# howardlau1999/pytorch-ddp-template

Measured on NVIDIA H100. Metric: samples/sec (whole box, device-timed, max over ranks) for ResNet-50 DDP at 1/2/4/8 H100, higher is better.
Workload: dtype bf16; 1 GPU; model=resnet50, global_batch=32, per_gpu_batch=32, image_size=224, parallelism=dp1, loss=mse(dense one-hot target), optimizer=sgd lr1e-3 + clip_grad_norm 1000 + linear warmup/decay, transport=single, cuda_graph=True

## Files before the change

### b200ddp/csrc/conv_wgmma.cu

```cuda
#include "conv.h"

#include <cuda.h>
#include <mutex>
#include <unordered_map>
#include <vector>

#include "drv.h"
#include "tc_primitives.cuh"

namespace b200 {
namespace {
using namespace tc;

constexpr int BLOCK_K = 64;
constexpr int UMMA_K = 16;
constexpr int kThreads = 256;
constexpr int kMmaWarps = 4;
constexpr int kMaxRing = 12;
constexpr int kSlabBytes = 128 * 128;
constexpr int kStagingBytes = 2 * kSlabBytes;
constexpr int kBarrierBytes = 1024;
constexpr int kTrStride = 36;
constexpr int kStatsScratchBytes = 4 * 32 * kTrStride * 4;
__host__ __device__ constexpr int acc_stride(int block_n) { return block_n + 8; }
__host__ __device__ constexpr int acc_bytes(int block_n) { return 128 * acc_stride(block_n) * 4; }

struct TapGemmParams {
  int M_total, Kc, Nc;
  int R, S, pad;
  int mirror;
  int mode;
  int H, W;
  int BH, BI, tiles_h, Wp;
  int num_m_tiles, num_n_tiles;
  int dense_rows;
  int a_chunk_bytes;
  int KC, TB;
  int s_stage_bytes, s_stages, b_slot_bytes, b_stages;
  uint32_t a_tx_bytes;
  int set_base_offset;
  int b_tap_stride;
  int row_mul;
  int b_resident;
  int chunk_stride;
  float* col_stats;
  const __nv_bfloat16* addend;
  const __nv_bfloat16* bn_x;
  const uint8_t* bn_mask;
  const float* bn_mean;
  const float* bn_rstd;
  long long* dbg;
};

__device__ __forceinline__ void tma_load_4d(const CUtensorMap* map, uint64_t* bar, void* smem, int c0, int c1, int c2, int c3) {
  asm volatile(
      "cp.async.bulk.tensor.4d.shared::cluster.global.mbarrier::complete_tx::bytes [%0], [%1, {%3, %4, %5, %6}], [%2];"
      ::"r"(smem_u32(smem)), "l"(reinterpret_cast<uint64_t>(map)), "r"(smem_u32(bar)), "r"(c0), "r"(c1), "r"(c2), "r"(c3) : "memory");
}
__device__ __forceinline__ void bulk_wait_read_all() { asm volatile("cp.async.bulk.wait_group.read 0;" ::: "memory"); }
__device__ __forceinline__ void epi_bar_sync() { asm volatile("bar.sync 1, 128;" ::: "memory"); }

__device__ __forceinline__ uint64_t make_desc_rowoff(uint32_t addr, uint32_t lbo, uint32_t sbo, int set_base_offset) {
  uint64_t d = make_smem_desc(addr, lbo, sbo);
  if (set_base_offset) d |= (uint64_t)((addr >> 7) & 7u) << 49;
  return d;
}

__device__ __forceinline__ bool acc_row_to_dense(const TapGemmParams& p, int i, int* dense) {
  if (p.mode == 2) {
    const int h = i / p.Wp, w = i - h * p.Wp;
    *dense = h * p.W + w;
    return h < p.BH && w < p.W;
  }
  *dense = i;
  return i < p.dense_rows;
}

__device__ __forceinline__ float warp_column_sum32(const float* v, float* tr, int lane) {
#pragma unroll
  for (int q = 0; q < 8; ++q)
    *reinterpret_cast<float4*>(tr + lane * kTrStride + 4 * q) = make_float4(v[4 * q], v[4 * q + 1], v[4 * q + 2], v[4 * q + 3]);
  __syncwarp();
  float s = 0.f;
#pragma unroll
  for (int r = 0; r < 32; ++r) s += tr[r * kTrStride + lane];
  __syncwarp();
  return s;
}

__device__ __forceinline__ bool elect_one() {
  uint32_t pred;
  asm volatile("{\n\t.reg .pred P;\n\telect.sync _|P, 0xFFFFFFFF;\n\tselp.u32 %0, 1, 0, P;\n\t}" : "=r"(pred));
  return pred != 0;
}

template <int BLOCK_N, bool B_MN, int EPI>
__global__ void __launch_bounds__(kThreads, 1)
conv_tap_gemm_kernel(const __grid_constant__ CUtensorMap map_a, const __grid_constant__ CUtensorMap map_b,
                     const __grid_constant__ CUtensorMap map_d, const TapGemmParams p) {
  constexpr int kBBytes = BLOCK_N * BLOCK_K * 2;
  constexpr int kAccStride = acc_stride(BLOCK_N);
  extern __shared__ uint8_t smem_raw[];
  uint8_t* smem = reinterpret_cast<uint8_t*>((reinterpret_cast<uintptr_t>(smem_raw) + 1023) & ~uintptr_t(1023));
  uint8_t* s_ring = smem;
  uint8_t* b_ring = s_ring + p.s_stages * p.s_stage_bytes;
  uint8_t* staging = b_ring + p.b_stages * p.b_slot_bytes;
  [[maybe_unused]] float* stats_scratch = reinterpret_cast<float*>(staging + kStagingBytes);
  float* acc_smem = reinterpret_cast<float*>(staging + kStagingBytes + (EPI != 0 ? kStatsScratchBytes : 0));
  uint64_t* s_full = reinterpret_cast<uint64_t*>(reinterpret_cast<uint8_t*>(acc_smem) + acc_bytes(BLOCK_N));
  uint64_t* s_empty = s_full + kMaxRing;
  uint64_t* b_full = s_empty + kMaxRing;
  uint64_t* b_empty = b_full + kMaxRing;

  const int warp = threadIdx.x >> 5, lane = threadIdx.x & 31;
  const long long t_begin = clock64();
  const int num_tiles = p.num_m_tiles * p.num_n_tiles;
  const int cblocks = p.Kc / BLOCK_K;
  const int taps = p.R * p.S;
  const int chunks_per_tile = cblocks * taps;

  if (warp == 0 && lane == 0) { tma_prefetch_desc(&map_a); tma_prefetch_desc(&map_b); tma_prefetch_desc(&map_d); }
  if (warp == 1) {
    if (lane < kMaxRing) {
      mbar_init(&s_full[lane], (p.mode == 2 || p.b_resident) ? 1 : 2); mbar_init(&s_empty[lane], kMmaWarps);
      mbar_init(&b_full[lane], 1); mbar_init(&b_empty[lane], kMmaWarps);
    }
    asm volatile("fence.mbarrier_init.release.cluster;" ::: "memory");
  }
  __syncthreads();
#define B200_T0 if (dbg) t = clock64();
#define B200_T1(acc) if (dbg) acc += clock64() - t;

  if (warp == 0 || warp == 3) {
    const bool is_a = (warp == 0);
    int ss = 0, bs = 0;
    uint32_t sph = 0, bph = 0;
    long long d_w = 0, d_i = 0, t = 0;
    const bool dbg = p.dbg != nullptr && blockIdx.x == 0;
    if constexpr (!B_MN) {
      if (!is_a && p.b_resident) {
        if (elect_one()) {
          mbar_expect_tx(&b_full[0], (uint32_t)chunks_per_tile * kBBytes);
          int cb_i = 0, r_i = 0, s_i = 0;
          for (int q = 0; q < chunks_per_tile; ++q) {
            tma_load_2d(&map_b, &b_full[0], b_ring + q * kBBytes, (r_i * p.S + s_i) * p.b_tap_stride + cb_i * BLOCK_K, 0);
            if (++s_i == p.S) { s_i = 0; if (++r_i == p.R) { r_i = 0; ++cb_i; } }
          }
        }
        __syncwarp();
      }
    }
    for (int tile = blockIdx.x; tile < num_tiles; tile += gridDim.x) {
      const int mt = tile / p.num_n_tiles, nt = tile - mt * p.num_n_tiles;
      const int n0 = nt * BLOCK_N;
      int img0 = 0, h0 = 0;
      if (p.mode != 0) { img0 = (mt / p.tiles_h) * p.BI; h0 = (mt % p.tiles_h) * p.BH; }
      if (p.mode != 2) {
        if (!is_a && p.b_resident) continue;
        int cb = 0, r = 0, sx = 0;
        for (int q0 = 0; q0 < chunks_per_tile; q0 += p.KC) {
          B200_T0 mbar_wait(&s_empty[ss], sph ^ 1); B200_T1(d_w)
          B200_T0
          if (elect_one()) {
            uint8_t* dst = s_ring + ss * p.s_stage_bytes;
            int cb_i = cb, r_i = r, s_i = sx;
            if (is_a) {
              mbar_expect_tx(&s_full[ss], (uint32_t)p.KC * p.a_tx_bytes);
              for (int j = 0; j < p.KC; ++j) {
                if (p.mode == 0) {
                  tma_load_4d(&map_a, &s_full[ss], dst, cb_i * BLOCK_K, mt * 128, 0, 0);
                } else {
                  const int dh = p.mirror ? p.pad - r_i : r_i - p.pad, dw = p.mirror ? p.pad - s_i : s_i - p.pad;
                  tma_load_4d(&map_a, &s_full[ss], dst, cb_i * BLOCK_K, dw, h0 * p.row_mul + dh, img0);
                }
                dst += p.chunk_stride;
                if (++s_i == p.S) { s_i = 0; if (++r_i == p.R) { r_i = 0; ++cb_i; } }
              }
            } else {
              mbar_expect_tx(&s_full[ss], (uint32_t)p.KC * kBBytes);
              for (int j = 0; j < p.KC; ++j) {
                uint8_t* sb = dst + p.a_chunk_bytes;
                const int bcol = (r_i * p.S + s_i) * p.b_tap_stride;
                if constexpr (!B_MN) {
                  tma_load_2d(&map_b, &s_full[ss], sb, bcol + cb_i * BLOCK_K, n0);
                } else {
#pragma unroll
                  for (int c = 0; c < BLOCK_N / 64; ++c)
                    tma_load_2d(&map_b, &s_full[ss], sb + c * (64 * BLOCK_K * 2), bcol + n0 + 64 * c, cb_i * BLOCK_K);
                }
                dst += p.chunk_stride;
                if (++s_i == p.S) { s_i = 0; if (++r_i == p.R) { r_i = 0; ++cb_i; } }
              }
            }
          }
          __syncwarp();
          for (int j = 0; j < p.KC; ++j) { if (++sx == p.S) { sx = 0; if (++r == p.R) { r = 0; ++cb; } } }
          if (++ss == p.s_stages) { ss = 0; sph ^= 1; }
          B200_T1(d_i)
        }
      } else if (is_a) {
        for (int cb = 0; cb < cblocks; ++cb) {
          B200_T0 mbar_wait(&s_empty[ss], sph ^ 1); B200_T1(d_w)
          B200_T0
          if (elect_one()) {
            mbar_expect_tx(&s_full[ss], p.a_tx_bytes);
            tma_load_4d(&map_a, &s_full[ss], s_ring + ss * p.s_stage_bytes, cb * BLOCK_K, -p.pad, h0 - p.pad, img0);
          }
          __syncwarp();
          if (++ss == p.s_stages) { ss = 0; sph ^= 1; }
          B200_T1(d_i)
        }
      } else {
        for (int cb = 0; cb < cblocks; ++cb) {
          for (int tap0 = 0; tap0 < taps; tap0 += p.TB) {
            B200_T0 mbar_wait(&b_empty[bs], bph ^ 1); B200_T1(d_w)
            B200_T0
            if (elect_one()) {
              mbar_expect_tx(&b_full[bs], (uint32_t)p.TB * kBBytes);
              for (int j = 0; j < p.TB; ++j) {
                uint8_t* sb = b_ring + bs * p.b_slot_bytes + j * kBBytes;
                const int bcol = (tap0 + j) * p.b_tap_stride;
                if constexpr (!B_MN) {
                  tma_load_2d(&map_b, &b_full[bs], sb, bcol + cb * BLOCK_K, n0);
                } else {
#pragma unroll
                  for (int c = 0; c < BLOCK_N / 64; ++c)
                    tma_load_2d(&map_b, &b_full[bs], sb + c * (64 * BLOCK_K * 2), bcol + n0 + 64 * c, cb * BLOCK_K);
                }
              }
            }
            __syncwarp();
            if (++bs == p.b_stages) { bs = 0; bph ^= 1; }
            B200_T1(d_i)
          }
        }
      }
    }
    if (dbg && lane == 0) { p.dbg[is_a ? 0 : 2] = d_w; p.dbg[is_a ? 1 : 3] = d_i; }
  } else if (warp >= 4) {
    constexpr int kTB = B_MN ? 1 : 0;
    constexpr uint32_t kLboB = B_MN ? BLOCK_K * 128 : 16;
    constexpr uint32_t kStepB = B_MN ? UMMA_K * 128 : UMMA_K * 2;
    constexpr uint64_t kHalfA = (64 * 128) >> 4;
    const uint64_t a_desc0 = make_smem_desc(smem_u32(s_ring), 16, 1024);
    const uint64_t b_desc_s0 = make_smem_desc(smem_u32(s_ring), kLboB, 1024);
    const uint64_t b_desc_b0 = make_smem_desc(smem_u32(b_ring), kLboB, 1024);
    const int ew = warp - 4;
    const bool t0 = (ew == 0 && lane == 0);
    int ss = 0, bs = 0;
    uint32_t sph = 0, bph = 0, slab = 0;
    long long d_wf = 0, d_mma = 0, d_ep = 0, t = 0;
    const bool dbg = p.dbg != nullptr && blockIdx.x == 0 && t0;
    [[maybe_unused]] float st_s[BLOCK_N / 32], st_q[BLOCK_N / 32];
    constexpr bool STATS = (EPI != 0);
    [[maybe_unused]] float* tr = stats_scratch + ew * (32 * kTrStride);
    if constexpr (STATS) {
#pragma unroll
      for (int i = 0; i < BLOCK_N / 32; ++i) { st_s[i] = 0.f; st_q[i] = 0.f; }
    }
    if (p.b_resident) mbar_wait(&b_full[0], 0);
    for (int tile = blockIdx.x; tile < num_tiles; tile += gridDim.x) {
      WgAcc<BLOCK_N> acc;
      uint32_t acc_on = 0;
      if (p.mode != 2) {
        for (int q0 = 0; q0 < chunks_per_tile; q0 += p.KC) {
          B200_T0 mbar_wait(&s_full[ss], sph); B200_T1(d_wf)
          B200_T0
          wgmma_fence();
          uint32_t off = (uint32_t)(ss * p.s_stage_bytes);
          for (int j = 0; j < p.KC; ++j) {
            const uint64_t da = a_desc0 + (uint64_t)(off >> 4);
            const uint64_t db = p.b_resident ? b_desc_b0 + (uint64_t)(((uint32_t)(q0 + j) * (uint32_t)kBBytes) >> 4)
                                             : b_desc_s0 + (uint64_t)((off + p.a_chunk_bytes) >> 4);
#pragma unroll
            for (int k = 0; k < BLOCK_K / UMMA_K; ++k) {
              const uint64_t dak = da + (uint64_t)(k * ((UMMA_K * 2) >> 4));
              wgmma_tile<BLOCK_N, 0, kTB>(acc, dak, dak + kHalfA, db + (uint64_t)(k * (kStepB >> 4)), acc_on);
              acc_on = 1;
            }
            off += (uint32_t)p.chunk_stride;
          }
          wgmma_commit();
          wgmma_wait<0>();
          __syncwarp();
          if (lane == 0) mbar_arrive(&s_empty[ss]);
          if (++ss == p.s_stages) { ss = 0; sph ^= 1; }
          B200_T1(d_mma)
        }
      } else {
        for (int cb = 0; cb < cblocks; ++cb) {
          B200_T0 mbar_wait(&s_full[ss], sph); B200_T1(d_wf)
          const uint32_t a_off = (uint32_t)(ss * p.s_stage_bytes);
          for (int tap0 = 0; tap0 < taps; tap0 += p.TB) {
            B200_T0 mbar_wait(&b_full[bs], bph); B200_T1(d_wf)
            B200_T0
            wgmma_fence();
            int r = tap0 / p.S, sx = tap0 - r * p.S;
            for (int j = 0; j < p.TB; ++j) {
              const int rr = p.mirror ? (p.R - 1 - r) : r, sc = p.mirror ? (p.S - 1 - sx) : sx;
              const uint64_t da = make_desc_rowoff(smem_u32(s_ring) + a_off + (uint32_t)(rr * p.Wp + sc) * 128u, 16, 1024, p.set_base_offset);
              const uint64_t db = b_desc_b0 + (uint64_t)((uint32_t)(bs * p.b_slot_bytes + j * kBBytes) >> 4);
#pragma unroll
              for (int k = 0; k < BLOCK_K / UMMA_K; ++k) {
                const uint64_t dak = da + (uint64_t)(k * ((UMMA_K * 2) >> 4));
                wgmma_tile<BLOCK_N, 0, kTB>(acc, dak, dak + kHalfA, db + (uint64_t)(k * (kStepB >> 4)), acc_on);
                acc_on = 1;
              }
              if (++sx == p.S) { sx = 0; ++r; }
            }
            wgmma_commit();
            wgmma_wait<0>();
            __syncwarp();
            if (lane == 0) {
              mbar_arrive(&b_empty[bs]);
              if (tap0 + p.TB >= taps) mbar_arrive(&s_empty[ss]);
            }
            if (++bs == p.b_stages) { bs = 0; bph ^= 1; }
            B200_T1(d_mma)
          }
          if (++ss == p.s_stages) { ss = 0; sph ^= 1; }
        }
      }
      B200_T0
      const int mt = tile / p.num_n_tiles, nt = tile - mt * p.num_n_tiles;
      const int n0 = nt * BLOCK_N;
      int row0;
      if (p.mode == 0) row0 = mt * 128;
      else row0 = (((mt / p.tiles_h) * p.BI) * p.H + (mt % p.tiles_h) * p.BH) * p.W;
      int dense;
      bool valid = acc_row_to_dense(p, ew * 32 + lane, &dense);
      valid = valid && (row0 + dense < p.M_total);
      wg_bar_sync();
      acc_to_smem<BLOCK_N>(acc, acc_smem, kAccStride, threadIdx.x - 128);
      wg_bar_sync();
#pragma unroll
      for (int c = 0; c < BLOCK_N; c += 64) {
        if (n0 + c >= p.Nc) break;
        uint8_t* buf = staging + (slab & 1u) * kSlabBytes;
        const uint32_t buf_s = smem_u32(buf);
#pragma unroll
        for (int half = 0; half < 2; ++half) {
          uint32_t rr[32];
          acc_row_ld32(acc_smem, kAccStride, ew * 32 + lane, c + 32 * half, rr);
          if constexpr (EPI == 1) {
            float sv[32], qv[32];
#pragma unroll
            for (int i = 0; i < 32; ++i) {
              const float v = __bfloat162float(__float2bfloat16_rn(__uint_as_float(rr[i])));
              sv[i] = valid ? v : 0.f;
              qv[i] = sv[i] * sv[i];
            }
            const float cs = warp_column_sum32(sv, tr, lane);
            const float cq = warp_column_sum32(qv, tr, lane);
            const int ci = (c >> 5) + half;
#pragma unroll
            for (int i = 0; i < BLOCK_N / 32; ++i)
              if (i == ci) { st_s[i] += cs; st_q[i] += cq; }
          }
          if constexpr (EPI == 2) {
            const int col0 = n0 + c + 32 * half;
            const size_t grow = (size_t)(row0 + dense);
            float v[32];
#pragma unroll
            for (int i = 0; i < 32; ++i) v[i] = __uint_as_float(rr[i]);
            if (p.addend != nullptr && valid) {
              const uint4* ap = reinterpret_cast<const uint4*>(p.addend + grow * p.Nc + col0);
#pragma unroll
              for (int q = 0; q < 4; ++q) {
                const uint4 raw = __ldg(ap + q);
                const __nv_bfloat162* h = reinterpret_cast<const __nv_bfloat162*>(&raw);
#pragma unroll
                for (int j = 0; j < 4; ++j) { const float2 f = __bfloat1622float2(h[j]); v[8 * q + 2 * j] += f.x; v[8 * q + 2 * j + 1] += f.y; }
              }
            }
#pragma unroll
            for (int i = 0; i < 32; ++i) { v[i] = __bfloat162float(__float2bfloat16_rn(v[i])); rr[i] = __float_as_uint(v[i]); }
            if (p.bn_x != nullptr) {
              float sv[32], qv[32];
              uint32_t mk = 0xffffffffu;
              float xv[32];
              if (valid) {
                const uint4* xp = reinterpret_cast<const uint4*>(p.bn_x + grow * p.Nc + col0);
#pragma unroll
                for (int q = 0; q < 4; ++q) {
                  const uint4 raw = __ldg(xp + q);
                  const __nv_bfloat162* h = reinterpret_cast<const __nv_bfloat162*>(&raw);
#pragma unroll
                  for (int j = 0; j < 4; ++j) { const float2 f = __bfloat1622float2(h[j]); xv[8 * q + 2 * j] = f.x; xv[8 * q + 2 * j + 1] = f.y; }
                }
                if (p.bn_mask != nullptr) mk = __ldg(reinterpret_cast<const uint32_t*>(p.bn_mask + grow * (size_t)(p.Nc >> 3) + (col0 >> 3)));
              } else {
                mk = 0u;
#pragma unroll
                for (int i = 0; i < 32; ++i) xv[i] = 0.f;
              }
              const float my_mean = (col0 + lane < p.Nc) ? __ldg(p.bn_mean + col0 + lane) : 0.f;
              const float my_rstd = (col0 + lane < p.Nc) ? __ldg(p.bn_rstd + col0 + lane) : 0.f;
#pragma unroll
              for (int i = 0; i < 32; ++i) {
                const float mean_i = __shfl_sync(0xffffffffu, my_mean, i), rstd_i = __shfl_sync(0xffffffffu, my_rstd, i);
                const float dyp = ((mk >> i) & 1u) ? v[i] : 0.f;
                sv[i] = dyp;
                qv[i] = dyp * (xv[i] - mean_i) * rstd_i;
              }
              const float cs = warp_column_sum32(sv, tr, lane);
              const float cq = warp_column_sum32(qv, tr, lane);
              const int ci = (c >> 5) + half;
#pragma unroll
              for (int i = 0; i < BLOCK_N / 32; ++i)
                if (i == ci) { st_s[i] += cs; st_q[i] += cq; }
            }
          }
          if (valid) {
#pragma unroll
            for (int q = 0; q < 4; ++q) {
              __nv_bfloat162 h[4];
#pragma unroll
              for (int j = 0; j < 4; ++j) h[j] = __floats2bfloat162_rn(__uint_as_float(rr[8 * q + 2 * j]), __uint_as_float(rr[8 * q + 2 * j + 1]));
              const int chunk = half * 4 + q;
              const uint32_t* w = reinterpret_cast<const uint32_t*>(h);
              asm volatile("st.shared.v4.b32 [%0], {%1, %2, %3, %4};"
                           ::"r"(buf_s + (uint32_t)(dense * 128 + ((chunk ^ (dense & 7)) << 4))), "r"(w[0]), "r"(w[1]), "r"(w[2]), "r"(w[3]) : "memory");
            }
          }
        }
        fence_async_smem();
        if (t0) bulk_wait_read_all();
        epi_bar_sync();
        if (t0) { tma_store_2d(&map_d, buf, n0 + c, row0); bulk_commit(); }
        ++slab;
      }
      B200_T1(d_ep)
    }
    if (dbg) { p.dbg[5] = d_wf; p.dbg[6] = d_mma; p.dbg[9] = d_ep; }
    if (STATS && p.col_stats != nullptr) {
      float* comb = stats_scratch;
      epi_bar_sync();
#pragma unroll
      for (int i = 0; i < BLOCK_N / 32; ++i) {
        comb[(ew * 2 + 0) * BLOCK_N + 32 * i + lane] = st_s[i];
        comb[(ew * 2 + 1) * BLOCK_N + 32 * i + lane] = st_q[i];
      }
      epi_bar_sync();
      const int nt = blockIdx.x % p.num_n_tiles;
      const size_t g = (size_t)(blockIdx.x / p.num_n_tiles), G = (size_t)(gridDim.x / p.num_n_tiles);
      for (int j = ew * 32 + lane; j < 2 * BLOCK_N; j += 128) {
        const int which = j / BLOCK_N, cc = j - which * BLOCK_N;
        const int col = nt * BLOCK_N + cc;
        if (col < p.Nc) {
          const float v = ((comb[(0 * 2 + which) * BLOCK_N + cc] + comb[(1 * 2 + which) * BLOCK_N + cc]) + comb[(2 * 2 + which) * BLOCK_N + cc]) +
                          comb[(3 * 2 + which) * BLOCK_N + cc];
          p.col_stats[((size_t)which * G + g) * p.Nc + col] = v;
        }
      }
    }
    if (t0) bulk_wait_all();
  }

  __syncthreads();
  if (p.dbg != nullptr && blockIdx.x == 0 && threadIdx.x == 0) p.dbg[10] = clock64() - t_begin;
}
#undef B200_T0
#undef B200_T1

struct MapKey {
  const void* ptr; uint64_t d[4]; uint64_t s[3]; uint32_t b[4]; int rank;
  bool operator==(const MapKey& o) const {
    if (ptr != o.ptr || rank != o.rank) return false;
    for (int i = 0; i < 4; ++i) if (d[i] != o.d[i] || b[i] != o.b[i]) return false;
    for (int i = 0; i < 3; ++i) if (s[i] != o.s[i]) return false;
    return true;
  }
};
struct MapKeyHash {
  size_t operator()(const MapKey& k) const {
    size_t h = std::hash<const void*>()(k.ptr) ^ (size_t)k.rank;
    for (int i = 0; i < 4; ++i) h = (h * 1000003u) ^ (size_t)k.d[i] ^ ((size_t)k.b[i] << 20);
    for (int i = 0; i < 3; ++i) h = (h * 1000003u) ^ (size_t)k.s[i];
    return h;
  }
};

}

CUtensorMap conv_encode_map(const void* ptr, int rank, const uint64_t* dims, const uint64_t* strides, const uint32_t* box) {
  static std::mutex mu;
  static std::unordered_map<MapKey, CUtensorMap, MapKeyHash> cache;
  MapKey key{};
  key.ptr = ptr; key.rank = rank;
  for (int i = 0; i < rank; ++i) { key.d[i] = dims[i]; key.b[i] = box[i]; }
  for (int i = 0; i + 1 < rank; ++i) key.s[i] = strides[i];
  {
    std::lock_guard<std::mutex> g(mu);
    auto it = cache.find(key);
    if (it != cache.end()) return it->second;
  }
  auto& drv = Driver::get();
  if (!drv.TensorMapEncodeTiled) throw std::runtime_error("conv: cuTensorMapEncodeTiled unavailable");
  static thread_local bool ctx_bound = false;
  if (!ctx_bound) { B200_CUDA_CHECK(cudaFree(nullptr)); ctx_bound = true; }
  CUtensorMap map;
  cuuint64_t d[4], s[3];
  cuuint32_t b[4], es[4] = {1, 1, 1, 1};
  for (int i = 0; i < rank; ++i) { d[i] = dims[i]; b[i] = box[i]; }
  for (int i = 0; i + 1 < rank; ++i) s[i] = strides[i];
  B200_DRV_CHECK(drv.TensorMapEncodeTiled(&map, CU_TENSOR_MAP_DATA_TYPE_BFLOAT16, rank, const_cast<void*>(ptr), d, s, b, es,
                                          CU_TENSOR_MAP_INTERLEAVE_NONE, CU_TENSOR_MAP_SWIZZLE_128B, CU_TENSOR_MAP_L2_PROMOTION_L2_256B,
                                          CU_TENSOR_MAP_FLOAT_OOB_FILL_NONE));
  std::lock_guard<std::mutex> g(mu);
  if (cache.size() > 8192) cache.clear();
  cache.emplace(key, map);
  return map;
}

bool conv_tile_plan(int N, int H, int W, int R, int S, int want_mode, ConvTilePlan* plan) {
  ConvTilePlan pl;
  const int taps = R * S;
  if (taps == 1) {
    if (want_mode > 0) return false;
    pl.mode = 0;
    pl.num_m_tiles = ceil_div((long long)N * H * W, 128);
    pl.dense_rows = 128; pl.acc_rows = 128; pl.a_rows = 128;
    *plan = pl;
    return true;
  }
  if (R != 3 || S != 3) return false;
  auto halo = [&]() {
    const int Wp = W + 2;
    int bh = 0;
    for (int d = 1; d <= H; ++d)
      if (H % d == 0 && d * Wp <= 128 && (d + 2) * Wp <= 256 * 1) bh = d;
    if (bh == 0 || Wp > 256 || bh + 2 > 256) return false;
    pl.mode = 2; pl.BH = bh; pl.BI = 1; pl.tiles_h = H / bh; pl.Wp = Wp;
    pl.num_m_tiles = N * pl.tiles_h;
    pl.dense_rows = bh * W; pl.acc_rows = bh * Wp; pl.a_rows = (bh + 2) * Wp;
    return true;
  };
  auto patch = [&]() {
    if (W > 128) return false;
    int bh = 0;
    for (int d = 1; d <= H; ++d)
      if (H % d == 0 && W * d <= 128) bh = d;
    if (bh == 0) return false;
    int bi = 1;
    if (bh == H)
      for (int d = 1; d <= N; ++d)
        if (N % d == 0 && W * H * d <= 128) bi = d;
    pl.mode = 1; pl.BH = bh; pl.BI = bi; pl.tiles_h = H / bh; pl.Wp = W;
    pl.num_m_tiles = (N / bi) * pl.tiles_h;
    pl.dense_rows = W * bh * bi; pl.acc_rows = pl.dense_rows; pl.a_rows = pl.dense_rows;
    return true;
  };
  bool ok;
  if (want_mode == 1) ok = patch();
  else if (want_mode == 2) ok = halo();
  else ok = halo() || patch();
  if (!ok) return false;
  *plan = pl;
  return true;
}

int conv_grid_size(int num_m_tiles, int num_n_tiles, bool stats) {
  const long long tiles = (long long)num_m_tiles * num_n_tiles;
  int grid = tiles < kNumSMs ? (int)tiles : kNumSMs;
  if (stats && num_n_tiles > 1) {
    grid = (grid / num_n_tiles) * num_n_tiles;
    if (grid < num_n_tiles) grid = num_n_tiles;
  }
  return grid;
}

int conv_pick_block_n(int Nc, int num_m_tiles, int want) {
  (void)num_m_tiles;
  if (want == 256) return 128;
  if (want != 0) return want;
  return Nc % 128 != 0 ? 64 : 128;
}

int conv_stat_groups(int N, int H, int W, int Cin, int Cout, int R, int S, const ConvLaunchCfg& cfg) {
  ConvTilePlan pl;
  int mode = cfg.mode;
  if (mode < 0 && R == 3) mode = (Cin == 64) ? 2 : 1;
  if (!conv_tile_plan(N, H, W, R, S, mode, &pl)) return 0;
  const int bn = conv_pick_block_n(Cout, pl.num_m_tiles, cfg.block_n);
  const int nn = ceil_div(Cout, bn);
  return conv_grid_size(pl.num_m_tiles, nn, true) / nn;
}

namespace {

template <int BLOCK_N, bool B_MN, int EPI>
void launch_variant(const CUtensorMap& ma, const CUtensorMap& mb, const CUtensorMap& md, TapGemmParams p, int want_kc, cudaStream_t stream) {
  constexpr int kBBytes = BLOCK_N * BLOCK_K * 2;
  const int budget = 227 * 1024 - kStagingBytes - kBarrierBytes - 1024 - (EPI != 0 ? kStatsScratchBytes : 0) - acc_bytes(BLOCK_N);
  const int taps = p.R * p.S;
  if (p.mode != 2) {
    const int chunks_per_tile = (p.Kc / BLOCK_K) * taps;
    if (p.b_resident && (B_MN || p.num_n_tiles != 1)) throw std::runtime_error("conv: a resident filter needs a K-major filter and one n-tile");
    p.chunk_stride = p.a_chunk_bytes + (p.b_resident ? 0 : kBBytes);
    p.b_slot_bytes = p.b_resident ? chunks_per_tile * kBBytes : 0;
    p.b_stages = p.b_resident ? 1 : 0;
    const int chunk = p.chunk_stride;
    const int ring_budget = budget - p.b_stages * p.b_slot_bytes;
    int kc = want_kc > 0 ? want_kc : 2;
    while (kc > 1 && (chunks_per_tile % kc != 0 || ring_budget / (kc * chunk) < 3)) --kc;
    p.KC = kc; p.TB = 1;
    p.s_stage_bytes = kc * chunk;
    p.s_stages = ring_budget / p.s_stage_bytes;
    if (p.s_stages > kMaxRing) p.s_stages = kMaxRing;
    if (p.s_stages < 2) throw std::runtime_error("conv: shared memory budget exceeded");
  } else {
    p.KC = 1; p.chunk_stride = 0; p.b_resident = 0;
    p.s_stage_bytes = p.a_chunk_bytes;
    int s_st = 0, b_st = 0;
    for (int tb = 3; tb >= 1; tb -= 2) {
      if (tb == 3 && (3 * kBBytes > 48 * 1024 || taps % 3 != 0)) continue;
      p.TB = tb;
      p.b_slot_bytes = p.TB * kBBytes;
      const int groups = taps / p.TB;
      s_st = budget / (p.s_stage_bytes + groups * p.b_slot_bytes);
      if (s_st < 2) s_st = 2;
      if (s_st > kMaxRing) s_st = kMaxRing;
      b_st = (budget - s_st * p.s_stage_bytes) / p.b_slot_bytes;
      if (b_st > kMaxRing) b_st = kMaxRing;
      if (b_st >= 2) break;
    }
    if (b_st < 2) throw std::runtime_error("conv: shared memory budget exceeded");
    p.s_stages = s_st; p.b_stages = b_st;
  }
  const int smem = p.s_stages * p.s_stage_bytes + p.b_stages * p.b_slot_bytes + kStagingBytes + kBarrierBytes + 1024 + (EPI != 0 ? kStatsScratchBytes : 0) +
                   acc_bytes(BLOCK_N);
  auto kernel = conv_tap_gemm_kernel<BLOCK_N, B_MN, EPI>;
  static std::atomic<unsigned long long> configured{0};
  ensure_max_dynamic_smem(kernel, 227 * 1024, configured);
  const int grid = conv_grid_size(p.num_m_tiles, p.num_n_tiles, EPI != 0);
  kernel<<<grid, kThreads, smem, stream>>>(ma, mb, md, p);
  B200_CUDA_CHECK(cudaGetLastError()); B200_COUNT_LAUNCH(1);
}

}

void launch_conv_tap_gemm(const void* a, const void* w, void* d, int N, int H, int W, int Cin, int Cout, int R, int S, bool dgrad,
                          const ConvLaunchCfg& cfg, float* col_stats, cudaStream_t stream, const ConvBwdFusion* fuse) {
  const int Kc = dgrad ? Cout : Cin, Nc = dgrad ? Cin : Cout;
  if (Kc % BLOCK_K != 0 || Nc % 64 != 0) throw std::runtime_error("conv: channel counts must be multiples of 64");
  if (R != S || (R != 1 && R != 3)) throw std::runtime_error("conv: 1x1 or 3x3 filters");
  if (dgrad && fuse == nullptr && col_stats != nullptr) throw std::runtime_error("conv: column statistics ride on the forward pass only");
  if (fuse != nullptr && !dgrad) throw std::runtime_error("conv: the BatchNorm-backward fusion rides on the data gradient");
  if (fuse != nullptr && fuse->bn_x != nullptr && col_stats == nullptr) throw std::runtime_error("conv: fused BatchNorm backward needs the partial-sum workspace");
  ConvTilePlan pl;
  int mode = cfg.mode;
  if (mode < 0 && R == 3) mode = (Kc == 64) ? 2 : 1;
  if (!conv_tile_plan(N, H, W, R, S, mode, &pl)) throw std::runtime_error("conv: no tile plan for this geometry");
  const long long M_total = (long long)N * H * W;
  TapGemmParams p{};
  p.M_total = (int)M_total; p.Kc = Kc; p.Nc = Nc;
  p.R = R; p.S = S; p.pad = (R - 1) / 2;
  p.mirror = dgrad ? 1 : 0;
  p.mode = pl.mode;
  p.H = H; p.W = W; p.BH = pl.BH; p.BI = pl.BI; p.tiles_h = pl.tiles_h; p.Wp = pl.Wp;
  p.num_m_tiles = pl.num_m_tiles;
  p.dense_rows = pl.dense_rows;
  p.a_tx_bytes = (uint32_t)(pl.a_rows * 128);
  p.a_chunk_bytes = ((pl.a_rows * 128 + 1023) / 1024) * 1024;
  if (p.a_chunk_bytes < 128 * 128) p.a_chunk_bytes = 128 * 128;
  p.set_base_offset = cfg.set_base_offset;
  p.b_tap_stride = Cin;
  p.row_mul = 1;
  p.b_resident = 0;
  p.col_stats = col_stats;
  p.addend = fuse ? reinterpret_cast<const __nv_bfloat16*>(fuse->addend) : nullptr;
  p.bn_x = fuse ? reinterpret_cast<const __nv_bfloat16*>(fuse->bn_x) : nullptr;
  p.bn_mask = fuse ? reinterpret_cast<const uint8_t*>(fuse->bn_mask) : nullptr;
  p.bn_mean = fuse ? fuse->bn_mean : nullptr;
  p.bn_rstd = fuse ? fuse->bn_rstd : nullptr;
  p.dbg = reinterpret_cast<long long*>(cfg.debug_counters);
  const int block_n = conv_pick_block_n(Nc, pl.num_m_tiles, cfg.block_n);
  if (block_n != 64 && block_n != 128) throw std::runtime_error("conv: block_n must be 0 (auto), 64, 128 or 256 (runs as two 128-wide n-tiles)");
  p.num_n_tiles = ceil_div(Nc, block_n);

  CUtensorMap ma;
  if (pl.mode == 0) {
    uint64_t dm[4] = {(uint64_t)Kc, (uint64_t)M_total, 1, 1};
    uint64_t st[3] = {(uint64_t)Kc * 2, (uint64_t)Kc * 2 * (uint64_t)M_total, (uint64_t)Kc * 2 * (uint64_t)M_total};
    uint32_t bx[4] = {64, 128, 1, 1};
    ma = conv_encode_map(a, 4, dm, st, bx);
  } else {
    uint64_t dm[4] = {(uint64_t)Kc, (uint64_t)W, (uint64_t)H, (uint64_t)N};
    uint64_t st[3] = {(uint64_t)Kc * 2, (uint64_t)W * Kc * 2, (uint64_t)H * W * Kc * 2};
    uint32_t bx[4] = {64, (uint32_t)(pl.mode == 2 ? pl.Wp : W), (uint32_t)(pl.mode == 2 ? pl.BH + 2 : pl.BH), (uint32_t)pl.BI};
    ma = conv_encode_map(a, 4, dm, st, bx);
  }
  CUtensorMap mb;
  {
    uint64_t dm[2] = {(uint64_t)R * S * Cin, (uint64_t)Cout};
    uint64_t st[1] = {(uint64_t)R * S * Cin * 2};
    uint32_t bx[2] = {64, (uint32_t)(dgrad ? 64 : block_n)};
    mb = conv_encode_map(w, 2, dm, st, bx);
  }
  CUtensorMap md;
  {
    uint64_t dm[2] = {(uint64_t)Nc, (uint64_t)M_total};
    uint64_t st[1] = {(uint64_t)Nc * 2};
    uint32_t bx[2] = {64, (uint32_t)pl.dense_rows};
    md = conv_encode_map(d, 2, dm, st, bx);
  }
#define B200_CONV_DISPATCH(BN)                                                                         \
  if (block_n == BN) {                                                                                 \
    if (dgrad && fuse != nullptr) launch_variant<BN, true, 2>(ma, mb, md, p, cfg.kc, stream);          \
    else if (dgrad) launch_variant<BN, true, 0>(ma, mb, md, p, cfg.kc, stream);                        \
    else if (col_stats != nullptr) launch_variant<BN, false, 1>(ma, mb, md, p, cfg.kc, stream);        \
    else launch_variant<BN, false, 0>(ma, mb, md, p, cfg.kc, stream);                                  \
    return;                                                                                            \
  }
  B200_CONV_DISPATCH(64)
  B200_CONV_DISPATCH(128)
#undef B200_CONV_DISPATCH
}

int stem_stat_groups(int N, int H, int W) {
  StemGeom g;
  if (!stem_geom(H, W, &g)) return 0;
  return conv_grid_size(N * g.Ho, 1, true);
}

void launch_stem_conv_fprop(const void* xp, const void* w2, void* y, int N, int H, int W, int Cout, float* col_stats, bool resident_filter,
                            void* debug_counters, cudaStream_t stream) {
  StemGeom g;
  if (!stem_geom(H, W, &g)) throw std::runtime_error("stem conv: unsupported image size");
  if (Cout != 64) throw std::runtime_error("stem conv: 64 output channels");
  const long long M_total = (long long)N * g.Ho * g.Wo;
  TapGemmParams p{};
  p.M_total = (int)M_total; p.Kc = 64; p.Nc = Cout;
  p.R = kStemTaps; p.S = 1; p.pad = 0; p.mirror = 0;
  p.mode = 1;
  p.H = g.Ho; p.W = g.Wo; p.BH = 1; p.BI = 1; p.tiles_h = g.Ho; p.Wp = g.Wo;
  p.num_m_tiles = N * g.Ho;
  p.num_n_tiles = 1;
  p.dense_rows = g.Wo;
  p.a_tx_bytes = (uint32_t)(g.Wo * 128);
  p.a_chunk_bytes = 128 * 128;
  p.b_tap_stride = 64;
  p.row_mul = 1;
  p.b_resident = resident_filter ? 1 : 0;
  p.col_stats = col_stats;
  p.dbg = reinterpret_cast<long long*>(debug_counters);
  const uint64_t row_pitch = (uint64_t)g.Wp * 16;
  CUtensorMap ma, mb, md;
  {
    uint64_t dm[4] = {64, (uint64_t)g.Wo, (uint64_t)g.Hp2, (uint64_t)N};
    uint64_t st[3] = {32, row_pitch, row_pitch * (uint64_t)g.Hp2};
    uint32_t bx[4] = {64, (uint32_t)g.Wo, 1, 1};
    ma = conv_encode_map(xp, 4, dm, st, bx);
  }
  {
    uint64_t dm[2] = {(uint64_t)kStemK, (uint64_t)Cout};
    uint64_t st[1] = {(uint64_t)kStemK * 2};
    uint32_t bx[2] = {64, 64};
    mb = conv_encode_map(w2, 2, dm, st, bx);
  }
  {
    uint64_t dm[2] = {(uint64_t)Cout, (uint64_t)M_total};
    uint64_t st[1] = {(uint64_t)Cout * 2};
    uint32_t bx[2] = {64, (uint32_t)g.Wo};
    md = conv_encode_map(y, 2, dm, st, bx);
  }
  if (col_stats != nullptr) launch_variant<64, false, 1>(ma, mb, md, p, 0, stream);
  else launch_variant<64, false, 0>(ma, mb, md, p, 0, stream);
}

}
```

### b200ddp/csrc/conv_wgrad_wgmma.cu

```cuda
#include "conv.h"

#include <cuda.h>

#include "drv.h"
#include "tc_primitives.cuh"

namespace b200 {

CUtensorMap conv_encode_map(const void* ptr, int rank, const uint64_t* dims, const uint64_t* strides, const uint32_t* box);

namespace {
using namespace tc;

constexpr int UMMA_K = 16;
constexpr int kThreads = 256;
constexpr int kMmaWarps = 4;
constexpr int kMaxRing = 12;
constexpr int kBarrierBytes = 1024;

struct WgradParams {
  int Cout, Cin, R, S, pad;
  int mode;
  int H, W, BH, BI, tiles_h;
  int row_mul;
  int KB;
  int num_kblocks;
  int MB, TG, tile_n;
  int m_groups, n_tiles, tap_groups, split;
  int a_slot_bytes, b_slot_bytes, a_stages, b_stages;
  float* partial;
};

__device__ __forceinline__ void tma_load_4d(const CUtensorMap* map, uint64_t* bar, void* smem, int c0, int c1, int c2, int c3) {
  asm volatile(
      "cp.async.bulk.tensor.4d.shared::cluster.global.mbarrier::complete_tx::bytes [%0], [%1, {%3, %4, %5, %6}], [%2];"
      ::"r"(smem_u32(smem)), "l"(reinterpret_cast<uint64_t>(map)), "r"(smem_u32(bar)), "r"(c0), "r"(c1), "r"(c2), "r"(c3) : "memory");
}

__device__ __forceinline__ bool elect_one() {
  uint32_t pred;
  asm volatile("{\n\t.reg .pred P;\n\telect.sync _|P, 0xFFFFFFFF;\n\tselp.u32 %0, 1, 0, P;\n\t}" : "=r"(pred));
  return pred != 0;
}

template <int N>
__device__ __forceinline__ void store_half_rows(const float (&h)[N / 2], float* out, size_t ld, int rows_valid, int cols_valid, bool zero, int wg_thread) {
  const int r0 = (wg_thread >> 5) * 16 + ((wg_thread & 31) >> 2), c0 = 2 * (wg_thread & 3);
#pragma unroll
  for (int j = 0; j < N / 8; ++j) {
#pragma unroll
    for (int hi = 0; hi < 2; ++hi) {
      const int r = r0 + 8 * hi, c = 8 * j + c0;
      if (r < rows_valid && c < cols_valid)
        *reinterpret_cast<float2*>(out + (size_t)r * ld + c) = zero ? make_float2(0.f, 0.f) : make_float2(h[4 * j + 2 * hi], h[4 * j + 2 * hi + 1]);
    }
  }
}

template <int TILE_N>
__global__ void __launch_bounds__(kThreads, 1)
conv_wgrad_kernel(const __grid_constant__ CUtensorMap map_dy, const __grid_constant__ CUtensorMap map_x, const WgradParams p) {
  extern __shared__ uint8_t smem_raw[];
  uint8_t* smem = reinterpret_cast<uint8_t*>((reinterpret_cast<uintptr_t>(smem_raw) + 1023) & ~uintptr_t(1023));
  uint8_t* a_ring = smem;
  uint8_t* b_ring = a_ring + p.a_stages * p.a_slot_bytes;
  uint64_t* a_full = reinterpret_cast<uint64_t*>(b_ring + p.b_stages * p.b_slot_bytes);
  uint64_t* a_empty = a_full + kMaxRing;
  uint64_t* b_full = a_empty + kMaxRing;
  uint64_t* b_empty = b_full + kMaxRing;

  const int warp = threadIdx.x >> 5, lane = threadIdx.x & 31;
  const int unit = blockIdx.x;
  const int grp = unit / p.split, sp = unit - grp * p.split;
  const int tg = grp % p.tap_groups;
  const int nt = (grp / p.tap_groups) % p.n_tiles;
  const int mg = grp / (p.tap_groups * p.n_tiles);
  const int taps = p.R * p.S;
  const int tap0 = tg * p.TG;
  const int ntaps = min(p.TG, taps - tap0);
  const int co0 = mg * p.MB * 128;
  const int ci0 = nt * p.tile_n;
  const int kb0 = (int)(((long long)p.num_kblocks * sp) / p.split);
  const int kb1 = (int)(((long long)p.num_kblocks * (sp + 1)) / p.split);
  const int chunk_bytes = p.KB * 128;
  const int a_chunks = p.MB * 2, b_chunks = p.tile_n / 64;

  if (warp == 0 && lane == 0) { tma_prefetch_desc(&map_dy); tma_prefetch_desc(&map_x); }
  if (warp == 1) {
    if (lane < kMaxRing) { mbar_init(&a_full[lane], 1); mbar_init(&a_empty[lane], kMmaWarps); mbar_init(&b_full[lane], 1); mbar_init(&b_empty[lane], kMmaWarps); }
    asm volatile("fence.mbarrier_init.release.cluster;" ::: "memory");
  }
  __syncthreads();

  if (warp == 0) {
    int as = 0;
    uint32_t aph = 0;
    for (int kb = kb0; kb < kb1; ++kb) {
      int c1 = 0, c2 = 0, c3 = 0;
      if (p.mode == 0) c1 = kb * p.KB;
      else { c3 = (kb / p.tiles_h) * p.BI; c2 = (kb % p.tiles_h) * p.BH; }
      mbar_wait(&a_empty[as], aph ^ 1);
      if (elect_one()) {
        mbar_expect_tx(&a_full[as], (uint32_t)(a_chunks * chunk_bytes));
        for (int j = 0; j < a_chunks; ++j)
          tma_load_4d(&map_dy, &a_full[as], a_ring + as * p.a_slot_bytes + j * chunk_bytes, co0 + 64 * j, c1, c2, c3);
      }
      __syncwarp();
      if (++as == p.a_stages) { as = 0; aph ^= 1; }
    }
  } else if (warp == 3) {
    int bs = 0;
    uint32_t bph = 0;
    for (int kb = kb0; kb < kb1; ++kb) {
      int c1 = 0, c2 = 0, c3 = 0;
      if (p.mode == 0) c1 = kb * p.KB;
      else { c3 = (kb / p.tiles_h) * p.BI; c2 = (kb % p.tiles_h) * p.BH; }
      int r = tap0 / p.S, sx = tap0 - r * p.S;
      for (int t = 0; t < ntaps; ++t) {
        mbar_wait(&b_empty[bs], bph ^ 1);
        if (elect_one()) {
          mbar_expect_tx(&b_full[bs], (uint32_t)(b_chunks * chunk_bytes));
          for (int j = 0; j < b_chunks; ++j)
            tma_load_4d(&map_x, &b_full[bs], b_ring + bs * p.b_slot_bytes + j * chunk_bytes, ci0 + 64 * j,
                        p.mode == 0 ? c1 : sx - p.pad, p.mode == 0 ? 0 : c2 * p.row_mul + r - p.pad, c3);
        }
        __syncwarp();
        if (++sx == p.S) { sx = 0; ++r; }
        if (++bs == p.b_stages) { bs = 0; bph ^= 1; }
      }
    }
  } else if (warp >= 4) {
    const uint32_t lbo = (uint32_t)chunk_bytes;
    const int ksteps = p.KB / UMMA_K;
    const uint64_t a_desc0 = make_smem_desc(smem_u32(a_ring), lbo, 1024);
    const uint64_t b_desc0 = make_smem_desc(smem_u32(b_ring), lbo, 1024);
    const uint64_t half_a = (uint64_t)(chunk_bytes >> 4);
    WgAcc<TILE_N> acc;
    int as = 0, bs = 0;
    uint32_t aph = 0, bph = 0;
    for (int kb = kb0; kb < kb1; ++kb) {
      mbar_wait(&a_full[as], aph);
      for (int t = 0; t < ntaps; ++t) {
        mbar_wait(&b_full[bs], bph);
        wgmma_fence();
        const uint64_t da0 = a_desc0 + (uint64_t)((uint32_t)(as * p.a_slot_bytes) >> 4);
        const uint64_t db0 = b_desc0 + (uint64_t)((uint32_t)(bs * p.b_slot_bytes) >> 4);
        for (int k = 0; k < ksteps; ++k) {
          const uint64_t step = (uint64_t)(k * ((UMMA_K * 128) >> 4));
          wgmma_tile<TILE_N, 1, 1>(acc, da0 + step, da0 + half_a + step, db0 + step, (kb != kb0 || k != 0) ? 1u : 0u);
        }
        wgmma_commit();
        wgmma_wait<0>();
        __syncwarp();
        if (lane == 0) {
          mbar_arrive(&b_empty[bs]);
          if (t == ntaps - 1) mbar_arrive(&a_empty[as]);
        }
        if (++bs == p.b_stages) { bs = 0; bph ^= 1; }
      }
      if (++as == p.a_stages) { as = 0; aph ^= 1; }
    }
    const int row_len = taps * p.Cin;
    float* out = p.partial + (size_t)sp * p.Cout * row_len + (size_t)co0 * row_len + (size_t)tap0 * p.Cin + ci0;
#pragma unroll
    for (int half = 0; half < 2; ++half)
      store_half_rows<TILE_N>(acc.h[half], out + (size_t)(64 * half) * row_len, (size_t)row_len, p.Cout - co0 - 64 * half, p.Cin - ci0,
                              kb1 <= kb0, threadIdx.x - 128);
  }
}

__global__ void __launch_bounds__(256) conv_wgrad_reduce_kernel(const float* __restrict__ partial, __nv_bfloat16* __restrict__ out, size_t n, int split) {
  __shared__ float sm[8][32][9];
  const int v = threadIdx.x & 31, sl = threadIdx.x >> 5;
  const size_t e = ((size_t)blockIdx.x * 32 + v) * 8;
  float acc[8] = {0.f, 0.f, 0.f, 0.f, 0.f, 0.f, 0.f, 0.f};
  if (e < n) {
#pragma unroll 2
    for (int s = sl; s < split; s += 8) {
      const float4 lo = __ldcg(reinterpret_cast<const float4*>(partial + (size_t)s * n + e));
      const float4 hi = __ldcg(reinterpret_cast<const float4*>(partial + (size_t)s * n + e + 4));
      acc[0] += lo.x; acc[1] += lo.y; acc[2] += lo.z; acc[3] += lo.w;
      acc[4] += hi.x; acc[5] += hi.y; acc[6] += hi.z; acc[7] += hi.w;
    }
  }
#pragma unroll
  for (int i = 0; i < 8; ++i) sm[sl][v][i] = acc[i];
  __syncthreads();
  if (sl == 0 && e < n) {
#pragma unroll
    for (int j = 1; j < 8; ++j)
#pragma unroll
      for (int i = 0; i < 8; ++i) acc[i] += sm[j][v][i];
    *reinterpret_cast<Bf16x8*>(out + e) = pack8(acc);
  }
}

struct WgradPlan {
  WgradParams p;
  int smem;
  int grid;
};

bool wgrad_plan(int N, int H, int W, int Cin, int Cout, int R, int S, const WgradCfg& cfg, WgradPlan* out) {
  if (Cin % 64 != 0 || Cout % 64 != 0 || R != S || (R != 1 && R != 3)) return false;
  WgradParams p{};
  p.Cout = Cout; p.Cin = Cin; p.R = R; p.S = S; p.pad = (R - 1) / 2;
  p.H = H; p.W = W; p.row_mul = 1;
  const int taps = R * S;
  if (taps == 1) {
    p.mode = 0; p.KB = 64;
    p.num_kblocks = ceil_div((long long)N * H * W, p.KB);
    p.BH = p.BI = p.tiles_h = 0;
  } else {
    p.mode = 1;
    int bh = 0, bi = 1;
    for (int d = 1; d <= 16 && bh == 0; ++d) {
      for (int i = 1; i <= (d >= H ? 4 : 1); ++i) {
        const int kb = W * d * i;
        if (kb % 16 == 0 && kb >= 96 && kb <= 128) { bh = d; bi = i; break; }
      }
    }
    if (bh == 0) {
      for (int d = 1; d <= H + 15 && bh == 0; ++d)
        if ((W * d) % 16 == 0 && W * d <= 128) bh = d;
      if (bh == 0) return false;
    }
    if (bi > 1 && N % bi != 0) return false;
    p.BH = bh; p.BI = bi; p.tiles_h = ceil_div(H, bh);
    p.KB = W * bh * bi;
    p.num_kblocks = (N / bi) * p.tiles_h;
  }
  const int MB = 1, TG = 1;
  int tile_n = Cin < 128 ? Cin : 128;
  if (cfg.tile_m > 0 && cfg.tile_m != 128) return false;
  if (cfg.tile_n > 0) tile_n = cfg.tile_n;
  if ((tile_n != 64 && tile_n != 128) || tile_n > Cin) return false;
  p.MB = MB; p.TG = TG; p.tile_n = tile_n;
  p.m_groups = ceil_div(Cout, 128 * MB);
  p.n_tiles = ceil_div(Cin, tile_n);
  p.tap_groups = ceil_div(taps, TG);
  const int groups = p.m_groups * p.n_tiles * p.tap_groups;
  int split = cfg.split > 0 ? cfg.split : kNumSMs / groups;
  if (split < 1) split = 1;
  if (split > p.num_kblocks) split = p.num_kblocks;
  p.split = split;
  const int chunk = p.KB * 128;
  p.a_slot_bytes = MB * 2 * chunk;
  p.b_slot_bytes = (tile_n / 64) * chunk;
  const int budget = 227 * 1024 - kBarrierBytes - 1024;
  int ast = budget / (p.a_slot_bytes + TG * p.b_slot_bytes);
  if (ast < 1) ast = 1;
  if (ast > kMaxRing) ast = kMaxRing;
  int bst = (budget - ast * p.a_slot_bytes) / p.b_slot_bytes;
  if (bst > kMaxRing) bst = kMaxRing;
  if (bst < 1) return false;
  p.a_stages = ast;
  p.b_stages = bst;
  out->p = p;
  out->smem = p.a_stages * p.a_slot_bytes + p.b_stages * p.b_slot_bytes + kBarrierBytes + 1024;
  out->grid = groups * split;
  return true;
}

void launch_wgrad_kernel(const CUtensorMap& mdy, const CUtensorMap& mx, const WgradPlan& pl, cudaStream_t stream) {
  if (pl.p.tile_n == 64) {
    static std::atomic<unsigned long long> configured{0};
    ensure_max_dynamic_smem(conv_wgrad_kernel<64>, 227 * 1024, configured);
    conv_wgrad_kernel<64><<<pl.grid, kThreads, pl.smem, stream>>>(mdy, mx, pl.p);
  } else {
    static std::atomic<unsigned long long> configured{0};
    ensure_max_dynamic_smem(conv_wgrad_kernel<128>, 227 * 1024, configured);
    conv_wgrad_kernel<128><<<pl.grid, kThreads, pl.smem, stream>>>(mdy, mx, pl.p);
  }
}

}

size_t conv_wgrad_workspace_floats(int N, int H, int W, int Cin, int Cout, int R, int S, const WgradCfg& cfg) {
  WgradPlan pl;
  if (!wgrad_plan(N, H, W, Cin, Cout, R, S, cfg, &pl)) return 0;
  return (size_t)pl.p.split * Cout * R * S * Cin;
}

void launch_conv_wgrad(const void* dy, const void* x, void* dw, int N, int H, int W, int Cin, int Cout, int R, int S,
                       const WgradCfg& cfg, float* workspace, cudaStream_t stream) {
  WgradPlan pl;
  if (!wgrad_plan(N, H, W, Cin, Cout, R, S, cfg, &pl)) throw std::runtime_error("conv wgrad: unsupported geometry / tiling");
  WgradParams& p = pl.p;
  p.partial = workspace;
  const long long M_total = (long long)N * H * W;
  CUtensorMap mdy, mx;
  if (p.mode == 0) {
    uint64_t dd[4] = {(uint64_t)Cout, (uint64_t)M_total, 1, 1};
    uint64_t ds[3] = {(uint64_t)Cout * 2, (uint64_t)Cout * 2 * (uint64_t)M_total, (uint64_t)Cout * 2 * (uint64_t)M_total};
    uint32_t bx[4] = {64, (uint32_t)p.KB, 1, 1};
    mdy = conv_encode_map(dy, 4, dd, ds, bx);
    uint64_t xd[4] = {(uint64_t)Cin, (uint64_t)M_total, 1, 1};
    uint64_t xs[3] = {(uint64_t)Cin * 2, (uint64_t)Cin * 2 * (uint64_t)M_total, (uint64_t)Cin * 2 * (uint64_t)M_total};
    mx = conv_encode_map(x, 4, xd, xs, bx);
  } else {
    uint32_t bx[4] = {64, (uint32_t)W, (uint32_t)p.BH, (uint32_t)p.BI};
    uint64_t dd[4] = {(uint64_t)Cout, (uint64_t)W, (uint64_t)H, (uint64_t)N};
    uint64_t ds[3] = {(uint64_t)Cout * 2, (uint64_t)W * Cout * 2, (uint64_t)H * W * Cout * 2};
    mdy = conv_encode_map(dy, 4, dd, ds, bx);
    uint64_t xd[4] = {(uint64_t)Cin, (uint64_t)W, (uint64_t)H, (uint64_t)N};
    uint64_t xs[3] = {(uint64_t)Cin * 2, (uint64_t)W * Cin * 2, (uint64_t)H * W * Cin * 2};
    mx = conv_encode_map(x, 4, xd, xs, bx);
  }
  launch_wgrad_kernel(mdy, mx, pl, stream);
  B200_CUDA_CHECK(cudaGetLastError());
  const size_t n = (size_t)Cout * R * S * Cin;
  conv_wgrad_reduce_kernel<<<(unsigned)((n / 8 + 31) / 32), 256, 0, stream>>>(workspace, reinterpret_cast<__nv_bfloat16*>(dw), n, p.split);
  B200_CUDA_CHECK(cudaGetLastError()); B200_COUNT_LAUNCH(2);
}

namespace {

struct StemWgradParams {
  int KB;
  int Ho, num_kblocks, split, Cout;
  int chunk_bytes, a_stages, b_stages;
  float* partial;
};
constexpr int kStemGroups = kStemTaps / 2;

__global__ void __launch_bounds__(kThreads, 1)
stem_wgrad_kernel(const __grid_constant__ CUtensorMap map_x, const __grid_constant__ CUtensorMap map_dy, const StemWgradParams p) {
  extern __shared__ uint8_t smem_raw[];
  uint8_t* smem = reinterpret_cast<uint8_t*>((reinterpret_cast<uintptr_t>(smem_raw) + 1023) & ~uintptr_t(1023));
  const int a_slot_bytes = 2 * p.chunk_bytes;
  uint8_t* a_ring = smem;
  uint8_t* b_ring = a_ring + p.a_stages * a_slot_bytes;
  uint64_t* a_full = reinterpret_cast<uint64_t*>(b_ring + p.b_stages * p.chunk_bytes);
  uint64_t* a_empty = a_full + kMaxRing;
  uint64_t* b_full = a_empty + kMaxRing;
  uint64_t* b_empty = b_full + kMaxRing;

  const int warp = threadIdx.x >> 5, lane = threadIdx.x & 31;
  const int sp = blockIdx.x;
  const int kb0 = (int)(((long long)p.num_kblocks * sp) / p.split);
  const int kb1 = (int)(((long long)p.num_kblocks * (sp + 1)) / p.split);

  if (warp == 0 && lane == 0) { tma_prefetch_desc(&map_x); tma_prefetch_desc(&map_dy); }
  if (warp == 1) {
    if (lane < kMaxRing) { mbar_init(&a_full[lane], 1); mbar_init(&a_empty[lane], kMmaWarps); mbar_init(&b_full[lane], 1); mbar_init(&b_empty[lane], kMmaWarps); }
    asm volatile("fence.mbarrier_init.release.cluster;" ::: "memory");
  }
  __syncthreads();

  if (warp == 0) {
    int as = 0;
    uint32_t aph = 0;
    for (int kb = kb0; kb < kb1; ++kb) {
      const int img = kb / p.Ho, oh = kb - img * p.Ho;
      for (int g = 0; g < kStemGroups; ++g) {
        mbar_wait(&a_empty[as], aph ^ 1);
        if (elect_one()) {
          uint8_t* dst = a_ring + as * a_slot_bytes;
          mbar_expect_tx(&a_full[as], (uint32_t)(2 * p.chunk_bytes));
          tma_load_4d(&map_x, &a_full[as], dst, 0, 0, oh + 2 * g, img);
          tma_load_4d(&map_x, &a_full[as], dst + p.chunk_bytes, 0, 0, oh + 2 * g + 1, img);
        }
        __syncwarp();
        if (++as == p.a_stages) { as = 0; aph ^= 1; }
      }
    }
  } else if (warp == 3) {
    int bs = 0;
    uint32_t bph = 0;
    for (int kb = kb0; kb < kb1; ++kb) {
      const int img = kb / p.Ho, oh = kb - img * p.Ho;
      mbar_wait(&b_empty[bs], bph ^ 1);
      if (elect_one()) {
        mbar_expect_tx(&b_full[bs], (uint32_t)p.chunk_bytes);
        tma_load_4d(&map_dy, &b_full[bs], b_ring + bs * p.chunk_bytes, 0, 0, oh, img);
      }
      __syncwarp();
      if (++bs == p.b_stages) { bs = 0; bph ^= 1; }
    }
  } else if (warp >= 4) {
    const int ksteps = p.KB / UMMA_K;
    const uint64_t a_desc0 = make_smem_desc(smem_u32(a_ring), (uint32_t)p.chunk_bytes, 1024);
    const uint64_t b_desc0 = make_smem_desc(smem_u32(b_ring), (uint32_t)p.chunk_bytes, 1024);
    const uint64_t half_a = (uint64_t)(p.chunk_bytes >> 4);
    WgAcc<64> acc[kStemGroups];
    int as = 0, bs = 0;
    uint32_t aph = 0, bph = 0;
    for (int kb = kb0; kb < kb1; ++kb) {
      mbar_wait(&b_full[bs], bph);
#pragma unroll
      for (int g = 0; g < kStemGroups; ++g) {
        mbar_wait(&a_full[as], aph);
        wgmma_fence();
        const uint64_t da0 = a_desc0 + (uint64_t)((uint32_t)(as * a_slot_bytes) >> 4);
        const uint64_t db0 = b_desc0 + (uint64_t)((uint32_t)(bs * p.chunk_bytes) >> 4);
        for (int k = 0; k < ksteps; ++k) {
          const uint64_t step = (uint64_t)(k * ((UMMA_K * 128) >> 4));
          wgmma_tile<64, 1, 1>(acc[g], da0 + step, da0 + half_a + step, db0 + step, (kb != kb0 || k != 0) ? 1u : 0u);
        }
        wgmma_commit();
        wgmma_wait<0>();
        __syncwarp();
        if (lane == 0) {
          mbar_arrive(&a_empty[as]);
          if (g == kStemGroups - 1) mbar_arrive(&b_empty[bs]);
        }
        if (++as == p.a_stages) { as = 0; aph ^= 1; }
      }
      if (++bs == p.b_stages) { bs = 0; bph ^= 1; }
    }
    float* base = p.partial + (size_t)sp * kStemK * p.Cout;
#pragma unroll
    for (int g = 0; g < kStemGroups; ++g)
#pragma unroll
      for (int half = 0; half < 2; ++half)
        store_half_rows<64>(acc[g].h[half], base + (size_t)(g * 128 + 64 * half) * p.Cout, (size_t)p.Cout, 64, p.Cout, kb1 <= kb0, threadIdx.x - 128);
  }
}

bool stem_generic_plan(int N, int H, int W, int Cout, WgradPlan* out) {
  StemGeom g;
  if (!stem_geom(H, W, &g) || Cout != 64) return false;
  WgradParams p{};
  p.Cout = Cout; p.Cin = 64; p.R = kStemTaps; p.S = 1; p.pad = 0;
  p.mode = 1; p.H = g.Ho; p.W = g.Wo; p.BH = 1; p.BI = 1; p.tiles_h = g.Ho; p.row_mul = 1;
  p.KB = g.Wo;
  p.num_kblocks = N * g.Ho;
  p.MB = 1; p.TG = 1; p.tile_n = 64;
  p.m_groups = 1; p.n_tiles = 1; p.tap_groups = kStemTaps;
  p.split = kNumSMs / kStemTaps;
  if (p.split > p.num_kblocks) p.split = p.num_kblocks;
  const int chunk = p.KB * 128;
  p.a_slot_bytes = 2 * chunk;
  p.b_slot_bytes = chunk;
  const int budget = 227 * 1024 - kBarrierBytes - 1024;
  p.a_stages = 3;
  int bst = (budget - p.a_stages * p.a_slot_bytes) / p.b_slot_bytes;
  if (bst > kMaxRing) bst = kMaxRing;
  if (bst < 2) return false;
  p.b_stages = bst;
  out->p = p;
  out->smem = p.a_stages * p.a_slot_bytes + p.b_stages * p.b_slot_bytes + kBarrierBytes + 1024;
  out->grid = p.tap_groups * p.split;
  return true;
}

bool stem_dedicated_plan(int N, int H, int W, int Cout, StemWgradParams* out, int* smem) {
  StemGeom g;
  if (!stem_geom(H, W, &g) || Cout != 64) return false;
  StemWgradParams p{};
  p.KB = g.Wo; p.Ho = g.Ho; p.Cout = Cout;
  p.num_kblocks = N * g.Ho;
  p.split = p.num_kblocks < kNumSMs ? p.num_kblocks : kNumSMs;
  p.chunk_bytes = p.KB * 128;
  const int budget = 227 * 1024 - kBarrierBytes - 1024;
  p.b_stages = 3;
  int ast = (budget - p.b_stages * p.chunk_bytes) / (2 * p.chunk_bytes);
  if (ast > kMaxRing) ast = kMaxRing;
  if (ast < 2) return false;
  p.a_stages = ast;
  *out = p;
  *smem = p.a_stages * 2 * p.chunk_bytes + p.b_stages * p.chunk_bytes + kBarrierBytes + 1024;
  return true;
}
}

size_t stem_wgrad_workspace_floats(int N, int H, int W, int Cout, int variant) {
  if (variant == 1) {
    WgradPlan pl;
    if (!stem_generic_plan(N, H, W, Cout, &pl)) return 0;
    return (size_t)pl.p.split * Cout * kStemK;
  }
  StemWgradParams p; int smem;
  if (!stem_dedicated_plan(N, H, W, Cout, &p, &smem)) return 0;
  return (size_t)p.split * Cout * kStemK;
}

void launch_stem_conv_wgrad(const void* dy, const void* xp, void* dw2, int N, int H, int W, int Cout, int variant, float* workspace,
                            cudaStream_t stream) {
  StemGeom g;
  if (!stem_geom(H, W, &g)) throw std::runtime_error("stem wgrad: unsupported geometry");
  CUtensorMap mdy, mx;
  uint32_t bx[4] = {64, (uint32_t)g.Wo, 1, 1};
  {
    uint64_t dd[4] = {(uint64_t)Cout, (uint64_t)g.Wo, (uint64_t)g.Ho, (uint64_t)N};
    uint64_t ds[3] = {(uint64_t)Cout * 2, (uint64_t)g.Wo * Cout * 2, (uint64_t)g.Ho * g.Wo * Cout * 2};
    mdy = conv_encode_map(dy, 4, dd, ds, bx);
  }
  {
    const uint64_t row_pitch = (uint64_t)g.Wp * 16;
    uint64_t xd[4] = {64, (uint64_t)g.Wo, (uint64_t)g.Hp2, (uint64_t)N};
    uint64_t xs[3] = {32, row_pitch, row_pitch * (uint64_t)g.Hp2};
    mx = conv_encode_map(xp, 4, xd, xs, bx);
  }
  const size_t n = (size_t)Cout * kStemK;
  int split = 0;
  if (variant == 1) {
    WgradPlan pl;
    if (!stem_generic_plan(N, H, W, Cout, &pl)) throw std::runtime_error("stem wgrad: unsupported geometry");
    pl.p.partial = workspace;
    launch_wgrad_kernel(mdy, mx, pl, stream);
    split = pl.p.split;
  } else {
    StemWgradParams p; int smem;
    if (!stem_dedicated_plan(N, H, W, Cout, &p, &smem)) throw std::runtime_error("stem wgrad: unsupported geometry");
    p.partial = workspace;
    static std::atomic<unsigned long long> configured{0};
    ensure_max_dynamic_smem(stem_wgrad_kernel, 227 * 1024, configured);
    stem_wgrad_kernel<<<p.split, kThreads, smem, stream>>>(mx, mdy, p);
    split = p.split;
  }
  B200_CUDA_CHECK(cudaGetLastError());
  conv_wgrad_reduce_kernel<<<(unsigned)((n / 8 + 31) / 32), 256, 0, stream>>>(workspace, reinterpret_cast<__nv_bfloat16*>(dw2), n, split);
  B200_CUDA_CHECK(cudaGetLastError()); B200_COUNT_LAUNCH(2);
}

}
```

### b200ddp/models/resnet.py

```python
from __future__ import annotations

import os
from typing import List

import torch
import torch.nn as nn

from ..ops import Conv3x3, FusedBatchNormAct2d, Linear, MaxPool3x3s2, PointwiseConv2d, StemConv7x7
from ..ops.bottleneck import bottleneck_forward, bottleneck_native_ok


class Bottleneck(nn.Module):
    expansion = 4

    def __init__(self, inplanes: int, planes: int, stride: int = 1, downsample: nn.Module | None = None):
        super().__init__()
        self.conv1 = PointwiseConv2d(inplanes, planes)
        self.bn1 = FusedBatchNormAct2d(planes, relu=True)
        self.conv2 = Conv3x3(planes, planes, stride=stride)
        self.bn2 = FusedBatchNormAct2d(planes, relu=True)
        self.conv3 = PointwiseConv2d(planes, planes * self.expansion)
        self.bn3 = FusedBatchNormAct2d(planes * self.expansion, relu=True)
        self.downsample = downsample

    def forward(self, x):
        if os.environ.get("B200DDP_BLOCK_FUSE", "0") == "1" and bottleneck_native_ok(self, x):
            return bottleneck_forward(self, x)
        if self.downsample is None:
            identity = x
        else:
            y, part = self.downsample[0].forward_with_stats(x)
            identity = self.downsample[1](y, partials=part)
        y, part = self.conv1.forward_with_stats(x)
        out = self.bn1(y, partials=part)
        y, part = self.conv2.forward_with_stats(out)
        out = self.bn2(y, partials=part)
        y, part = self.conv3.forward_with_stats(out)
        return self.bn3(y, residual=identity, partials=part)


class ResNet(nn.Module):
    def __init__(self, layers: List[int], num_classes: int = 1000, zero_init_residual: bool = False):
        super().__init__()
        self.inplanes = 64
        self.conv1 = StemConv7x7(3, 64)
        self.bn1 = FusedBatchNormAct2d(64, relu=True)
        self.maxpool = MaxPool3x3s2()
        self.layer1 = self._make_layer(64, layers[0], 1)
        self.layer2 = self._make_layer(128, layers[1], 2)
        self.layer3 = self._make_layer(256, layers[2], 2)
        self.layer4 = self._make_layer(512, layers[3], 2)
        self.avgpool = nn.AdaptiveAvgPool2d((1, 1))
        self.fc = Linear(512 * Bottleneck.expansion, num_classes)
        for m in self.modules():
            if isinstance(m, nn.Conv2d):
                nn.init.kaiming_normal_(m.weight, mode="fan_out", nonlinearity="relu")
            elif isinstance(m, nn.BatchNorm2d):
                nn.init.ones_(m.weight)
                nn.init.zeros_(m.bias)
        if zero_init_residual:
            for m in self.modules():
                if isinstance(m, Bottleneck):
                    nn.init.zeros_(m.bn3.weight)

    def _make_layer(self, planes: int, blocks: int, stride: int) -> nn.Sequential:
        downsample = None
        if stride != 1 or self.inplanes != planes * Bottleneck.expansion:
            downsample = nn.Sequential(PointwiseConv2d(self.inplanes, planes * Bottleneck.expansion, stride=stride),
                                       FusedBatchNormAct2d(planes * Bottleneck.expansion))
        mods = [Bottleneck(self.inplanes, planes, stride, downsample)]
        self.inplanes = planes * Bottleneck.expansion
        mods += [Bottleneck(self.inplanes, planes) for _ in range(1, blocks)]
        return nn.Sequential(*mods)

    def forward(self, x):
        if self.training:
            y, part = self.conv1.forward_with_stats(x)
        else:
            y, part = self.conv1(x), None
        x = self.maxpool(self.bn1(y, partials=part))
        x = self.layer4(self.layer3(self.layer2(self.layer1(x))))
        x = torch.flatten(self.avgpool(x), 1)
        return self.fc(x)


def resnet50(num_classes: int = 1000, **kw) -> ResNet:
    return ResNet([3, 4, 6, 3], num_classes, **kw)


def resnet152(num_classes: int = 1000, **kw) -> ResNet:
    return ResNet([3, 8, 36, 3], num_classes, **kw)
```

### b200ddp/ops/functional.py

```python
from __future__ import annotations

import math
import os
from typing import Optional

import torch
import torch.nn.functional as F

from .. import _ext

EPI_NONE, EPI_BIAS, EPI_BIAS_RELU, EPI_BIAS_GELU = 0, 1, 2, 3
_ACT_TO_EPI = {None: EPI_BIAS, "relu": EPI_BIAS_RELU, "gelu": EPI_BIAS_GELU}
_GELU_TANH = {"gelu": False, "gelu_tanh": True}


def _gelu_tanh_grad(p: torch.Tensor) -> torch.Tensor:
    k = math.sqrt(2.0 / math.pi)
    t = torch.tanh(k * (p + 0.044715 * p * p * p))
    return 0.5 * (1.0 + t) + 0.5 * p * (1.0 - t * t) * k * (1.0 + 3.0 * 0.044715 * p * p)


def _C():
    return _ext.get()


def _tc_ok(M: int, N: int, K: int) -> bool:
    return K % 8 == 0 and N % 8 == 0 and M % 8 == 0


class _LinearTC(torch.autograd.Function):

    @staticmethod
    def forward(ctx, x, weight, bias, activation):
        C = _C()
        x2 = x.reshape(-1, x.shape[-1])
        if not x2.is_contiguous():
            x2 = x2.contiguous()
        if bias is None and activation is not None:
            raise ValueError("fused activation needs a bias (use bias=True)")
        if activation in _GELU_TANH:
            pre = C.gemm_nt(x2, weight, bias, EPI_BIAS, None)
            y = C.gelu_fwd(pre, _GELU_TANH[activation])
            ctx.save_for_backward(x2, weight, pre)
        else:
            y = C.gemm_nt(x2, weight, bias, _ACT_TO_EPI[activation] if bias is not None else EPI_NONE, None)
            ctx.save_for_backward(x2, weight, y if activation == "relu" else None)
        ctx.activation = activation
        ctx.has_bias = bias is not None
        ctx.x_shape = x.shape
        return y.view(*x.shape[:-1], weight.shape[0])

    @staticmethod
    def backward(ctx, dy):
        C = _C()
        x2, weight, aux = ctx.saved_tensors
        dy2 = dy.reshape(-1, dy.shape[-1])
        if ctx.activation == "relu":
            dy2 = dy2 * (aux > 0).to(dy2.dtype)
        elif ctx.activation in _GELU_TANH:
            dy2 = C.gelu_bwd(dy2.contiguous(), aux, _GELU_TANH[ctx.activation])
        if not dy2.is_contiguous():
            dy2 = dy2.contiguous()
        dx = dw = db = None
        if ctx.needs_input_grad[0]:
            dx = C.gemm(dy2, weight, None, False, True, EPI_NONE, False, None).view(ctx.x_shape)
        if ctx.needs_input_grad[1]:
            dw = C.gemm(dy2, x2, None, True, True, EPI_NONE, False, None)
        if ctx.has_bias and ctx.needs_input_grad[2]:
            db = dy2.sum(0)
        return dx, dw, db, None


class _LinearSmall(torch.autograd.Function):

    @staticmethod
    def forward(ctx, x, weight, bias, relu):
        C = _C()
        xc = x.contiguous()
        y = C.small_linear_fwd(xc, weight.contiguous(), bias, bool(relu))
        ctx.save_for_backward(xc, weight, y)
        ctx.relu = bool(relu)
        ctx.has_bias = bias is not None
        return y

    @staticmethod
    def backward(ctx, dy):
        C = _C()
        x, weight, y = ctx.saved_tensors
        dx, dw, db = C.small_linear_bwd(dy, x, weight.contiguous(), y, ctx.relu, ctx.needs_input_grad[0], ctx.has_bias)
        return (dx if ctx.needs_input_grad[0] else None), dw, (db if ctx.has_bias else None), None


FP8_FORMATS = {"e4m3": (torch.float8_e4m3fn, 448.0), "e5m2": (torch.float8_e5m2, 57344.0)}


def fp8_scale(amax: float, fmt: str) -> float:
    fmax = FP8_FORMATS[fmt][1]
    if not (amax > 0.0) or not math.isfinite(amax):
        return 1.0
    ma, ea = math.frexp(amax)
    mf, ef = math.frexp(fmax)
    e = ef - ea - (1 if ma > mf else 0)
    return math.ldexp(1.0, min(max(e, -126), 127))


def fp8_quantize_reference(t: torch.Tensor, fmt: str):
    s = fp8_scale(float(t.detach().abs().max().float()) if t.numel() else 0.0, fmt)
    return (t.detach().float() * s).to(FP8_FORMATS[fmt][0]), s


def _fp8_round_trip(t: torch.Tensor, fmt: str) -> torch.Tensor:
    q, s = fp8_quantize_reference(t, fmt)
    return q.float() / s


def _fp8_check(x2: torch.Tensor, weight: torch.Tensor, bias: Optional[torch.Tensor], need_transpose_x: bool) -> None:
    M, K = x2.shape
    N = weight.shape[0]
    if x2.dtype != torch.bfloat16 or weight.dtype != torch.bfloat16 or (bias is not None and bias.dtype != torch.bfloat16):
        raise ValueError(f"fp8 linear on CUDA needs bf16 input, weight and bias, got {x2.dtype} x {weight.dtype} "
                         f"(input {tuple(x2.shape)}, weight {tuple(weight.shape)})")
    if K % 16 or N % 16:
        raise ValueError(f"fp8 linear needs in_features and out_features divisible by 16, got weight {tuple(weight.shape)}")
    if need_transpose_x and M % 16:
        raise ValueError(f"fp8 linear backward needs the row count divisible by 16 (the weight gradient reduces over rows "
                         f"of a transposed FP8 copy), got input {tuple(x2.shape)}")


class _LinearFP8(torch.autograd.Function):

    @staticmethod
    def forward(ctx, x, weight, bias, activation, grad_enabled):
        x2 = x.reshape(-1, x.shape[-1])
        if not x2.is_contiguous():
            x2 = x2.contiguous()
        if bias is None and activation is not None:
            raise ValueError("fused activation needs a bias (use bias=True)")
        need_dx, need_dw = grad_enabled and ctx.needs_input_grad[0], grad_enabled and ctx.needs_input_grad[1]
        ctx.activation = activation
        ctx.has_bias = bias is not None
        ctx.x_shape = x.shape
        if x.is_cuda:
            C = _C()
            _fp8_check(x2, weight, bias, need_dw)
            xq, xqt, xs, _ = C.fp8_quantize(x2, "e4m3", need_dw, False)
            wq, wqt, ws, _ = C.fp8_quantize(weight.contiguous(), "e4m3", need_dx, False)
            if activation in _GELU_TANH:
                pre = C.gemm_fp8(xq, wq, xs, ws, bias, EPI_BIAS)
                y = C.gelu_fwd(pre, _GELU_TANH[activation])
            else:
                pre = None
                y = C.gemm_fp8(xq, wq, xs, ws, bias, _ACT_TO_EPI[activation] if bias is not None else EPI_NONE)
                if activation == "relu":
                    pre = y
            ctx.save_for_backward(xqt, xs, wqt, ws, pre)
        else:
            xd = _fp8_round_trip(x2, "e4m3")
            wd = _fp8_round_trip(weight, "e4m3")
            acc = xd @ wd.t()
            if bias is not None:
                acc = acc + bias.float()
            pre = acc.to(x.dtype)
            if activation == "gelu":
                y = F.gelu(pre.float()).to(x.dtype)
            elif activation == "gelu_tanh":
                y = F.gelu(pre.float(), approximate="tanh").to(x.dtype)
            elif activation == "relu":
                y = F.relu(pre)
            else:
                y = pre
            ctx.save_for_backward(xd, wd, pre if activation is not None else None)
            ctx.dtypes = (x.dtype, weight.dtype, bias.dtype if bias is not None else None)
        return y.view(*x.shape[:-1], weight.shape[0])

    @staticmethod
    def backward(ctx, dy):
        dy2 = dy.reshape(-1, dy.shape[-1])
        dx = dw = db = None
        if dy.is_cuda:
            C = _C()
            xqt, xs, wqt, ws, aux = ctx.saved_tensors
            if ctx.activation == "relu":
                dy2 = dy2 * (aux > 0).to(dy2.dtype)
            elif ctx.activation in _GELU_TANH:
                dy2 = C.gelu_bwd(dy2.contiguous(), aux, _GELU_TANH[ctx.activation])
            if not dy2.is_contiguous():
                dy2 = dy2.contiguous()
            if dy2.shape[0] % 16:
                raise ValueError(f"fp8 linear backward needs the row count divisible by 16, got gradient {tuple(dy2.shape)}")
            need_db = ctx.has_bias and ctx.needs_input_grad[2]
            dyq, dyqt, dys, colsum = C.fp8_quantize(dy2, "e5m2", ctx.needs_input_grad[1], need_db)
            if ctx.needs_input_grad[0]:
                dx = C.gemm_fp8(dyq, wqt, dys, ws, None, EPI_NONE).view(ctx.x_shape)
            if ctx.needs_input_grad[1]:
                dw = C.gemm_fp8(dyqt, xqt, dys, xs, None, EPI_NONE)
            if need_db:
                db = colsum.to(dy.dtype)
        else:
            xd, wd, aux = ctx.saved_tensors
            x_dtype, w_dtype, b_dtype = ctx.dtypes
            if ctx.activation == "relu":
                dy2 = dy2 * (aux > 0).to(dy2.dtype)
            elif ctx.activation == "gelu":
                p = aux.float()
                dgelu = 0.5 * (1.0 + torch.erf(p * math.sqrt(0.5))) + p * torch.exp(-0.5 * p * p) / math.sqrt(2.0 * math.pi)
                dy2 = (dy2.float() * dgelu).to(dy.dtype)
            elif ctx.activation == "gelu_tanh":
                dy2 = (dy2.float() * _gelu_tanh_grad(aux.float())).to(dy.dtype)
            dyd = _fp8_round_trip(dy2, "e5m2")
            if ctx.needs_input_grad[0]:
                dx = (dyd @ wd).to(x_dtype).view(ctx.x_shape)
            if ctx.needs_input_grad[1]:
                dw = (dyd.t() @ xd).to(w_dtype)
            if ctx.has_bias and ctx.needs_input_grad[2]:
                db = dy2.float().sum(0).to(b_dtype)
        return dx, dw, db, None, None


def linear(x: torch.Tensor, weight: torch.Tensor, bias: Optional[torch.Tensor] = None,
           activation: Optional[str] = None, fp8: bool = False) -> torch.Tensor:
    if fp8:
        return _LinearFP8.apply(x, weight, bias, activation, torch.is_grad_enabled())
    if x.is_cuda:
        N, K = weight.shape
        M = x.numel() // K
        if x.dtype == torch.bfloat16 and weight.dtype == torch.bfloat16 and _tc_ok(M, N, K) \
                and (bias is not None or activation is None) and os.environ.get("B200DDP_DISABLE_TC", "0") != "1":
            return _LinearTC.apply(x, weight, bias, activation)
        if x.dtype == torch.float32 and weight.dtype == torch.float32 and N * (K + 1) * 4 <= 48 * 1024 and M * N * 4 <= 48 * 1024 \
                and activation in (None, "relu"):
            return _LinearSmall.apply(x, weight, bias, activation == "relu")
        _C()
        y = F.linear(x, weight, bias)
    else:
        y = F.linear(x, weight, bias)
    if activation == "relu":
        y = F.relu(y)
    elif activation == "gelu":
        y = F.gelu(y)
    elif activation == "gelu_tanh":
        y = F.gelu(y, approximate="tanh")
    return y


ATTENTION_HEAD_DIM = 64
ATTENTION_SEQ_MULTIPLE = 128


def _key_mask(seq_lens: torch.Tensor, S: int, device) -> torch.Tensor:
    lens = seq_lens.to(device=device, dtype=torch.long).clamp(0, S)
    return torch.arange(S, device=device)[None, :] < lens[:, None]


def attention_reference(qkv: torch.Tensor, seq_lens: torch.Tensor, heads: int) -> torch.Tensor:
    return _masked_attention_reference(qkv, _key_mask(seq_lens, qkv.shape[1], qkv.device)[:, None, None, :], heads)


def _masked_attention_reference(qkv: torch.Tensor, keep: torch.Tensor, heads: int) -> torch.Tensor:
    B, S, W = qkv.shape
    hidden = W // 3
    hd = hidden // heads
    ct = torch.promote_types(qkv.dtype, torch.float32)
    q, k, v = (t.to(ct).reshape(B, S, heads, hd).transpose(1, 2) for t in qkv.split(hidden, dim=-1))
    scores = (q @ k.transpose(-1, -2)) * (1.0 / math.sqrt(hd))
    p = torch.softmax(scores.masked_fill(~keep, torch.finfo(ct).min), dim=-1) * keep
    return (p @ v).transpose(1, 2).reshape(B, S, hidden).to(qkv.dtype)


def _attention_check(qkv: torch.Tensor, seq_lens: torch.Tensor, heads: int) -> None:
    _qkv_check(qkv, heads)
    B = qkv.shape[0]
    if seq_lens.dim() != 1 or seq_lens.shape[0] != B or seq_lens.is_floating_point() or seq_lens.is_complex():
        raise ValueError(f"attention needs integer seq_lens [B] = [{B}], got {seq_lens.dtype} {tuple(seq_lens.shape)}")


def _qkv_check(qkv: torch.Tensor, heads: int) -> None:
    if qkv.dim() != 3 or qkv.shape[-1] % 3:
        raise ValueError(f"attention needs qkv [B, S, 3 * hidden], got {tuple(qkv.shape)}")
    B, S, W = qkv.shape
    if heads < 1 or (W // 3) % heads or (W // 3) // heads != ATTENTION_HEAD_DIM:
        raise ValueError(f"attention on CUDA supports head dim {ATTENTION_HEAD_DIM} only, got hidden {W // 3} over {heads} heads")
    if qkv.dtype != torch.bfloat16:
        raise ValueError(f"attention on CUDA needs bf16 qkv, got {qkv.dtype}")
    if S % ATTENTION_SEQ_MULTIPLE or S == 0:
        raise ValueError(f"attention on CUDA needs the sequence length to be a multiple of {ATTENTION_SEQ_MULTIPLE}, got {S}")
    if not qkv.is_contiguous():
        raise ValueError("attention on CUDA needs a contiguous qkv (the fused projection's output)")


_ATTENTION_MODES = {
    "key_padding": ("attention_fwd", "attention_bwd", lambda: attention_reference),
    "packed": ("packed_attention_fwd", "packed_attention_bwd", lambda: packed_attention_reference),
    "causal": ("causal_attention_fwd", "causal_attention_bwd", lambda: causal_attention_reference),
}


class _Attention(torch.autograd.Function):

    @staticmethod
    def forward(ctx, qkv, mask, heads, mode):
        ctx.heads, ctx.mode = heads, mode
        if qkv.is_cuda:
            B, S, W = qkv.shape
            m = mask.to(device=qkv.device, dtype=torch.int32).contiguous()
            o, lse = getattr(_C(), _ATTENTION_MODES[mode][0])(qkv.view(B * S, W), m, heads)
            ctx.save_for_backward(qkv, o, lse, m)
            return o.view(B, S, W // 3)
        ctx.save_for_backward(qkv, mask)
        return _ATTENTION_MODES[mode][2]()(qkv, mask, heads)

    @staticmethod
    def backward(ctx, dy):
        if dy.is_cuda:
            qkv, o, lse, m = ctx.saved_tensors
            B, S, W = qkv.shape
            do = dy.reshape(B * S, W // 3).to(torch.bfloat16).contiguous()
            if do.data_ptr() % 16:
                do = do.clone()
            dqkv = getattr(_C(), _ATTENTION_MODES[ctx.mode][1])(do, qkv.view(B * S, W), o, lse, m, ctx.heads)
            return dqkv.view(B, S, W), None, None, None
        qkv, mask = ctx.saved_tensors
        ref = _ATTENTION_MODES[ctx.mode][2]()
        with torch.enable_grad():
            x = qkv.detach().requires_grad_(True)
            (g,) = torch.autograd.grad(ref(x, mask, ctx.heads), x, dy)
        return g, None, None, None


def attention(qkv: torch.Tensor, seq_lens: torch.Tensor, heads: int) -> torch.Tensor:
    if qkv.is_cuda:
        _attention_check(qkv, seq_lens, heads)
    return _Attention.apply(qkv, seq_lens, heads, "key_padding")


def document_bounds(input_ids: torch.Tensor, cls_token_id: Optional[int], pad_token_id: Optional[int]):
    B, S = input_ids.shape
    pos = torch.arange(S, device=input_ids.device).expand(B, S)
    if pad_token_id is None:
        lens = torch.full((B, 1), S, device=input_ids.device, dtype=torch.long)
    else:
        lens = (input_ids != pad_token_id).sum(1, keepdim=True)
    valid = pos < lens
    is_start = (pos == 0) if cls_token_id is None else (input_ids == cls_token_id) | (pos == 0)
    is_start = is_start & valid
    start = torch.where(is_start, pos, 0).cummax(1).values
    nxt = torch.where(is_start, pos, S)[:, 1:]
    nxt = torch.cat([nxt, torch.full((B, 1), S, device=pos.device, dtype=pos.dtype)], 1).flip(1).cummin(1).values.flip(1)
    end = torch.minimum(nxt, lens)
    bounds = torch.stack([torch.where(valid, start, 0), torch.where(valid, end, 0)], -1).to(torch.int32)
    return bounds, torch.where(valid, pos - start, 0)


def _bounds_mask(bounds: torch.Tensor, S: int, device) -> torch.Tensor:
    b = bounds.to(device=device, dtype=torch.long).reshape(-1, S, 2)
    start = b[..., 0].clamp(0, S)
    end = torch.maximum(b[..., 1].clamp(max=S), start)
    j = torch.arange(S, device=device)
    return (j >= start[..., None]) & (j < end[..., None])


def packed_attention_reference(qkv: torch.Tensor, bounds: torch.Tensor, heads: int) -> torch.Tensor:
    return _masked_attention_reference(qkv, _bounds_mask(bounds, qkv.shape[1], qkv.device)[:, None], heads)


def packed_attention(qkv: torch.Tensor, bounds: torch.Tensor, heads: int) -> torch.Tensor:
    if qkv.is_cuda:
        _qkv_check(qkv, heads)
        _bounds_check(qkv, bounds, "packed attention")
    return _Attention.apply(qkv, bounds, heads, "packed")


def _bounds_check(qkv: torch.Tensor, bounds: torch.Tensor, who: str) -> None:
    B, S = qkv.shape[:2]
    if tuple(bounds.shape) != (B, S, 2) or bounds.is_floating_point() or bounds.is_complex():
        raise ValueError(f"{who} needs integer bounds [B, S, 2] = [{B}, {S}, 2], got {bounds.dtype} {tuple(bounds.shape)}")


def _causal_mask(bounds: torch.Tensor, S: int, device) -> torch.Tensor:
    i = torch.arange(S, device=device)
    return _bounds_mask(bounds, S, device) & (i[None, :] <= i[:, None])


def causal_attention_reference(qkv: torch.Tensor, bounds: torch.Tensor, heads: int, kv_heads: Optional[int] = None) -> torch.Tensor:
    if kv_heads is not None and kv_heads != heads:
        qkv = _repeat_kv(qkv, heads, kv_heads)
    return _masked_attention_reference(qkv, _causal_mask(bounds, qkv.shape[1], qkv.device)[:, None], heads)


def _repeat_kv(qkv: torch.Tensor, heads: int, kv_heads: int) -> torch.Tensor:
    B, S, Wd = qkv.shape
    d = Wd // (heads + 2 * kv_heads)
    q, k, v = qkv.split([heads * d, kv_heads * d, kv_heads * d], dim=-1)
    rep = heads // kv_heads
    k, v = (t.reshape(B, S, kv_heads, 1, d).expand(B, S, kv_heads, rep, d).reshape(B, S, heads * d) for t in (k, v))
    return torch.cat([q, k, v], -1)


def _gqa_check(qkv: torch.Tensor, heads: int, kv_heads: int) -> None:
    if heads < 1 or kv_heads < 1 or heads % kv_heads:
        raise ValueError(f"grouped-query attention needs kv_heads dividing heads, got heads={heads}, kv_heads={kv_heads}")
    if qkv.dim() != 3 or qkv.shape[-1] != (heads + 2 * kv_heads) * ATTENTION_HEAD_DIM:
        raise ValueError(f"grouped-query attention on CUDA needs qkv [B, S, (heads + 2 * kv_heads) * {ATTENTION_HEAD_DIM}] = "
                         f"[B, S, {(heads + 2 * kv_heads) * ATTENTION_HEAD_DIM}], got {tuple(qkv.shape)}")
    if qkv.dtype != torch.bfloat16:
        raise ValueError(f"attention on CUDA needs bf16 qkv, got {qkv.dtype}")
    S = qkv.shape[1]
    if S % ATTENTION_SEQ_MULTIPLE or S == 0:
        raise ValueError(f"attention on CUDA needs the sequence length to be a multiple of {ATTENTION_SEQ_MULTIPLE}, got {S}")
    if not qkv.is_contiguous():
        raise ValueError("attention on CUDA needs a contiguous qkv (the fused projection's output)")


class _GqaAttention(torch.autograd.Function):

    @staticmethod
    def forward(ctx, qkv, bounds, heads, kv_heads):
        ctx.heads, ctx.kv_heads = heads, kv_heads
        if qkv.is_cuda:
            B, S, Wd = qkv.shape
            m = bounds.to(device=qkv.device, dtype=torch.int32).contiguous()
            o, lse = _C().causal_gqa_attention_fwd(qkv.view(B * S, Wd), m, heads, kv_heads)
            ctx.save_for_backward(qkv, o, lse, m)
            return o.view(B, S, heads * ATTENTION_HEAD_DIM)
        ctx.save_for_backward(qkv, bounds)
        return causal_attention_reference(qkv, bounds, heads, kv_heads)

    @staticmethod
    def backward(ctx, dy):
        if dy.is_cuda:
            qkv, o, lse, m = ctx.saved_tensors
            B, S, Wd = qkv.shape
            do = dy.reshape(B * S, -1).to(torch.bfloat16).contiguous()
            if do.data_ptr() % 16:
                do = do.clone()
            dqkv = _C().causal_gqa_attention_bwd(do, qkv.view(B * S, Wd), o, lse, m, ctx.heads, ctx.kv_heads)
            return dqkv.view(B, S, Wd), None, None, None
        qkv, bounds = ctx.saved_tensors
        with torch.enable_grad():
            x = qkv.detach().requires_grad_(True)
            (g,) = torch.autograd.grad(causal_attention_reference(x, bounds, ctx.heads, ctx.kv_heads), x, dy)
        return g, None, None, None


def causal_attention(qkv: torch.Tensor, bounds: torch.Tensor, heads: int, kv_heads: Optional[int] = None) -> torch.Tensor:
    if kv_heads is not None and kv_heads != heads:
        if qkv.is_cuda:
            _gqa_check(qkv, heads, kv_heads)
            _bounds_check(qkv, bounds, "causal attention")
        elif heads < 1 or kv_heads < 1 or heads % kv_heads or qkv.dim() != 3 or qkv.shape[-1] % (heads + 2 * kv_heads):
            raise ValueError(f"grouped-query attention needs kv_heads dividing heads and qkv [B, S, (heads + 2 * kv_heads) * d], "
                             f"got heads={heads}, kv_heads={kv_heads}, qkv {tuple(qkv.shape)}")
        return _GqaAttention.apply(qkv, bounds, heads, kv_heads)
    if qkv.is_cuda:
        _qkv_check(qkv, heads)
        _bounds_check(qkv, bounds, "causal attention")
    return _Attention.apply(qkv, bounds, heads, "causal")


def rotary_cos_sin(max_position: int, head_dim: int = ATTENTION_HEAD_DIM, theta: float = 10000.0) -> torch.Tensor:
    inv = theta ** (-torch.arange(0, head_dim, 2, dtype=torch.float64) / head_dim)
    ang = torch.arange(max_position, dtype=torch.float64)[:, None] * inv[None, :]
    return torch.stack([ang.cos(), ang.sin()], 1).float()


def _rotary_reference(qkv: torch.Tensor, position_ids: torch.Tensor, cos_sin: torch.Tensor, heads: int, kv_heads: int,
                      inverse: bool = False) -> torch.Tensor:
    B, S, Wd = qkv.shape
    d = Wd // (heads + 2 * kv_heads)
    half = d // 2
    ct = torch.promote_types(qkv.dtype, torch.float32)
    pos = position_ids.to(device=qkv.device, dtype=torch.long).reshape(B, S).clamp(0, cos_sin.shape[0] - 1)
    cs = cos_sin.to(device=qkv.device, dtype=ct)[pos]
    cos, sin = cs[:, :, None, 0], cs[:, :, None, 1]
    if inverse:
        sin = -sin
    qk, v = qkv.to(ct).split([(heads + kv_heads) * d, kv_heads * d], dim=-1)
    x = qk.reshape(B, S, heads + kv_heads, d)
    lo, hi = x[..., :half], x[..., half:]
    out = torch.cat([lo * cos - hi * sin, hi * cos + lo * sin], -1).reshape(B, S, -1)
    return torch.cat([out, v], -1).to(qkv.dtype)


class _Rotary(torch.autograd.Function):
    @staticmethod
    def forward(ctx, qkv, position_ids, cos_sin, heads, kv_heads):
        ctx.heads, ctx.kv_heads = heads, kv_heads
        if qkv.is_cuda:
            B, S, Wd = qkv.shape
            pos = position_ids.to(device=qkv.device, dtype=torch.int32).reshape(-1).contiguous()
            table = cos_sin.to(device=qkv.device, dtype=torch.float32).contiguous()
            ctx.save_for_backward(pos, table)
            return _C().rotary(qkv.reshape(B * S, Wd).contiguous(), pos, table, heads, kv_heads, False).view(B, S, Wd)
        ctx.save_for_backward(position_ids, cos_sin)
        return _rotary_reference(qkv, position_ids, cos_sin, heads, kv_heads)

    @staticmethod
    def backward(ctx, dy):
        pos, table = ctx.saved_tensors
        if dy.is_cuda:
            B, S, Wd = dy.shape
            dx = _C().rotary(dy.reshape(B * S, Wd).to(torch.bfloat16).contiguous(), pos, table, ctx.heads, ctx.kv_heads, True)
            return dx.view(B, S, Wd), None, None, None, None
        return _rotary_reference(dy, pos, table, ctx.heads, ctx.kv_heads, inverse=True), None, None, None, None


def rotary(qkv: torch.Tensor, position_ids: torch.Tensor, cos_sin: torch.Tensor, heads: int, kv_heads: int) -> torch.Tensor:
    if qkv.dim() != 3 or heads < 1 or kv_heads < 1 or qkv.shape[-1] % (heads + 2 * kv_heads) or \
            (qkv.shape[-1] // (heads + 2 * kv_heads)) % 2:
        raise ValueError(f"rotary needs qkv [B, S, (heads + 2 * kv_heads) * d] with an even d, got {tuple(qkv.shape)} for "
                         f"heads={heads}, kv_heads={kv_heads}")
    d = qkv.shape[-1] // (heads + 2 * kv_heads)
    if tuple(position_ids.shape) != tuple(qkv.shape[:2]) or position_ids.is_floating_point() or position_ids.is_complex():
        raise ValueError(f"rotary needs integer position_ids {tuple(qkv.shape[:2])}, got {position_ids.dtype} {tuple(position_ids.shape)}")
    if cos_sin.dim() != 3 or tuple(cos_sin.shape[1:]) != (2, d // 2) or cos_sin.shape[0] < 1:
        raise ValueError(f"rotary needs cos_sin [max_position, 2, {d // 2}], got {tuple(cos_sin.shape)}")
    if qkv.is_cuda and (qkv.dtype != torch.bfloat16 or d != ATTENTION_HEAD_DIM):
        raise ValueError(f"rotary on CUDA needs bf16 qkv and head dim {ATTENTION_HEAD_DIM}, got {qkv.dtype}, head dim {d}")
    return _Rotary.apply(qkv, position_ids, cos_sin, heads, kv_heads)


def _rms_norm_reference(x: torch.Tensor, weight: torch.Tensor, eps: float) -> torch.Tensor:
    xf = x.float()
    return (xf * torch.rsqrt(xf.pow(2).mean(-1, keepdim=True) + eps) * weight.float()).to(x.dtype)


class _RMSNormFused(torch.autograd.Function):
    @staticmethod
    def forward(ctx, x, weight, eps):
        xc = x.contiguous()
        y, rstd = _C().rmsnorm_fwd(xc, weight.contiguous(), float(eps))
        ctx.save_for_backward(xc, weight, rstd)
        return y

    @staticmethod
    def backward(ctx, dy):
        x, weight, rstd = ctx.saved_tensors
        dx, dw = _C().rmsnorm_bwd(dy.contiguous().to(x.dtype), x, weight.contiguous(), rstd)
        return dx, dw, None


def rms_norm(x: torch.Tensor, weight: torch.Tensor, eps: float = 1e-5) -> torch.Tensor:
    if x.dim() < 1 or weight.dim() != 1 or weight.shape[0] != x.shape[-1]:
        raise ValueError(f"rms_norm needs x [..., hidden] and weight [hidden], got {tuple(x.shape)} and {tuple(weight.shape)}")
    if x.is_cuda:
        n = x.shape[-1]
        if x.dtype not in (torch.float32, torch.bfloat16) or weight.dtype != x.dtype or n % 8 or n > 1024:
            raise ValueError(f"rms_norm on CUDA needs bf16 or fp32 x and weight of one dtype and hidden % 8 == 0, <= 1024; got "
                             f"{x.dtype} x {weight.dtype}, hidden {n}")
        if weight.device != x.device:
            raise ValueError(f"rms_norm needs the weight on x's device ({x.device}), got {weight.device}")
        return _RMSNormFused.apply(x, weight, eps)
    return _rms_norm_reference(x, weight, eps)


class _SwiGLU(torch.autograd.Function):
    @staticmethod
    def forward(ctx, gate_up):
        gu = gate_up.contiguous()
        ctx.save_for_backward(gu)
        return _C().swiglu_fwd(gu)

    @staticmethod
    def backward(ctx, dy):
        (gu,) = ctx.saved_tensors
        return _C().swiglu_bwd(dy.to(gu.dtype).contiguous(), gu)


def _swiglu_reference(gate_up: torch.Tensor) -> torch.Tensor:
    g, u = gate_up.float().chunk(2, dim=-1)
    return (F.silu(g) * u).to(gate_up.dtype)


def swiglu(gate_up: torch.Tensor) -> torch.Tensor:
    if gate_up.dim() < 1 or gate_up.shape[-1] % 2:
        raise ValueError(f"swiglu needs [..., 2 * I] (gate | up), got {tuple(gate_up.shape)}")
    if gate_up.is_cuda:
        if gate_up.dtype != torch.bfloat16 or (gate_up.shape[-1] // 2) % 8:
            raise ValueError(f"swiglu on CUDA needs bf16 and I % 8 == 0, got {gate_up.dtype} {tuple(gate_up.shape)}")
        return _SwiGLU.apply(gate_up)
    return _swiglu_reference(gate_up)


def _conv_policy() -> str:
    return os.environ.get("B200DDP_CONV", "auto")


def _fprop_native(cin: int, cout: int, k: int, pixels: int) -> bool:
    mode = _conv_policy()
    if mode == "native":
        return True
    if mode == "lib":
        return False
    return False


def _dgrad_native(cin: int, cout: int, k: int, pixels: int) -> bool:
    return _conv_policy() == "native"


def _wgrad_native(cin: int, cout: int, k: int, pixels: int) -> bool:
    mode = os.environ.get("B200DDP_CONV_WGRAD", "auto")
    if mode == "native":
        return True
    if mode == "lib" or _conv_policy() == "lib":
        return False
    if _conv_policy() == "native":
        return k == 1 and pixels >= 25088 and not (cin == 64 and cout == 64)
    return False


def conv_tc_supported(x: torch.Tensor, weight: torch.Tensor, stride: int, padding: int) -> bool:
    k = weight.shape[2]
    return (x.is_cuda and x.dtype == torch.bfloat16 and weight.dtype == torch.bfloat16 and x.dim() == 4 and stride == 1
            and weight.shape[2] == weight.shape[3] and k in (1, 3) and padding == (k - 1) // 2
            and x.shape[1] % 64 == 0 and weight.shape[0] % 64 == 0 and x.shape[3] + 2 <= 256 and _conv_policy() != "lib")


def conv_tc_wanted(x: torch.Tensor, weight: torch.Tensor, stride: int, padding: int) -> bool:
    if not conv_tc_supported(x, weight, stride, padding):
        return False
    n, cin, h, w = x.shape
    return _fprop_native(cin, weight.shape[0], weight.shape[2], n * h * w)


def _cl(t: torch.Tensor) -> torch.Tensor:
    return t if t.is_contiguous(memory_format=torch.channels_last) else t.contiguous(memory_format=torch.channels_last)


class _ConvTC(torch.autograd.Function):

    @staticmethod
    def forward(ctx, x, w, want_stats):
        C = _C()
        xc, wc = _cl(x), _cl(w)
        k = w.shape[2]
        y, st = C.conv_fprop(xc, wc, 1, (k - 1) // 2, -1, 0, 0, bool(want_stats))
        ctx.save_for_backward(xc, wc)
        ctx.k = k
        ctx.w_strides = w.stride()
        if want_stats:
            ctx.mark_non_differentiable(st)
            return y, st
        return y, None

    @staticmethod
    def backward(ctx, dy, _dstats):
        C = _C()
        x, w = ctx.saved_tensors
        k = ctx.k
        pad = (k - 1) // 2
        dyc = _cl(dy)
        dx = dw = None
        n, cin, h, wd = x.shape
        if ctx.needs_input_grad[0]:
            if _dgrad_native(cin, w.shape[0], k, n * h * wd):
                dx = C.conv_dgrad(dyc, w, 1, pad, -1, 0, 0)[0]
            else:
                dx = torch.ops.aten.convolution_backward(dyc, x, w, None, [1, 1], [pad, pad], [1, 1], False, [0, 0], 1,
                                                         [True, False, False])[0]
        if ctx.needs_input_grad[1]:
            if _wgrad_native(cin, w.shape[0], k, n * h * wd):
                dw = C.conv_wgrad(dyc, x, k, 1, pad, 0, 0, 0)
            else:
                dw = torch.ops.aten.convolution_backward(dyc, x, w, None, [1, 1], [pad, pad], [1, 1], False, [0, 0], 1,
                                                         [False, True, False])[1]
            if k == 1 and tuple(dw.stride()) != tuple(ctx.w_strides):
                dw = dw.as_strided(dw.shape, ctx.w_strides)
        return dx, dw, None


def conv2d_tc(x: torch.Tensor, weight: torch.Tensor, want_stats: bool = False):
    return _ConvTC.apply(x, weight, want_stats)


def _stem_policy() -> str:
    return os.environ.get("B200DDP_STEM", "native")


def stem_conv_supported(x: torch.Tensor, weight: torch.Tensor, stride, padding) -> bool:
    if _stem_policy() == "lib" or not (x.is_cuda and x.dim() == 4 and x.dtype == torch.bfloat16 and weight.dtype == torch.bfloat16):
        return False
    if tuple(weight.shape) != (64, 3, 7, 7) or tuple(stride) != (2, 2) or tuple(padding) != (3, 3) or x.shape[1] != 3:
        return False
    if x.requires_grad and torch.is_grad_enabled():
        return False
    if not (x.is_contiguous(memory_format=torch.channels_last) and weight.is_contiguous(memory_format=torch.channels_last)):
        return False
    return bool(_C().stem_conv_supported(int(x.shape[2]), int(x.shape[3])))


class _StemConv(torch.autograd.Function):

    @staticmethod
    def forward(ctx, x, w, want_stats):
        resident = os.environ.get("B200DDP_STEM_RESIDENT", "1") != "0"
        y, st, xp = _C().stem_conv_fprop(x, w, bool(want_stats), resident)
        ctx.save_for_backward(xp)
        ctx.hw = (int(x.shape[2]), int(x.shape[3]))
        ctx.w_strides = w.stride()
        if want_stats:
            ctx.mark_non_differentiable(st)
            return y, st
        return y, None

    @staticmethod
    def backward(ctx, dy, _dstats):
        (xp,) = ctx.saved_tensors
        dw = None
        if ctx.needs_input_grad[1]:
            variant = 1 if os.environ.get("B200DDP_STEM_WGRAD", "dedicated") == "generic" else 0
            dw = _C().stem_conv_wgrad(_cl(dy), xp, ctx.hw[0], ctx.hw[1], variant)
            if tuple(dw.stride()) != tuple(ctx.w_strides):
                dw = dw.as_strided(dw.shape, ctx.w_strides)
        return None, dw, None


def stem_conv(x: torch.Tensor, weight: torch.Tensor, want_stats: bool = False):
    return _StemConv.apply(x, weight, want_stats)


class _MSEFused(torch.autograd.Function):
    @staticmethod
    def forward(ctx, out, target):
        loss, dout = _C().mse_fwd_bwd(out.contiguous(), target.contiguous(), 1.0)
        ctx.save_for_backward(dout)
        return loss.to(out.dtype) if out.dtype != torch.float32 else loss

    @staticmethod
    def backward(ctx, g):
        (dout,) = ctx.saved_tensors
        return dout * g.to(dout.dtype), None


def mse_loss(out: torch.Tensor, target: torch.Tensor) -> torch.Tensor:
    if out.is_cuda and out.dtype in (torch.float32, torch.bfloat16) and out.dtype == target.dtype and out.shape == target.shape:
        return _MSEFused.apply(out, target)
    return F.mse_loss(out.float(), target.float())


class _XentFused(torch.autograd.Function):
    @staticmethod
    def forward(ctx, logits, targets, ignore_index):
        loss, dlogits = _C().xent_fwd_bwd(logits.contiguous(), targets.contiguous(), int(ignore_index), 1.0)
        ctx.save_for_backward(dlogits)
        return loss

    @staticmethod
    def backward(ctx, g):
        (dlogits,) = ctx.saved_tensors
        return dlogits * g.to(dlogits.dtype), None, None


def cross_entropy(logits: torch.Tensor, targets: torch.Tensor, ignore_index: int = -100) -> torch.Tensor:
    if logits.is_cuda and logits.dtype in (torch.float32, torch.bfloat16):
        flat = logits.reshape(-1, logits.shape[-1])
        return _XentFused.apply(flat, targets.reshape(-1), ignore_index)
    return F.cross_entropy(logits.reshape(-1, logits.shape[-1]).float(), targets.reshape(-1), ignore_index=ignore_index)


class _LayerNormFused(torch.autograd.Function):
    @staticmethod
    def forward(ctx, x, gamma, beta, eps):
        xc = x.contiguous()
        y, mean, rstd = _C().layernorm_fwd(xc, gamma.contiguous(), beta.contiguous(), float(eps))
        ctx.save_for_backward(xc, gamma, mean, rstd)
        return y

    @staticmethod
    def backward(ctx, dy):
        x, gamma, mean, rstd = ctx.saved_tensors
        dx, dgamma, dbeta = _C().layernorm_bwd(dy.contiguous(), x, gamma.contiguous(), mean, rstd)
        return dx, dgamma, dbeta, None


def layer_norm(x: torch.Tensor, gamma: torch.Tensor, beta: torch.Tensor, eps: float = 1e-5) -> torch.Tensor:
    if x.is_cuda and x.dtype in (torch.float32, torch.bfloat16) and gamma.dtype == x.dtype and x.shape[-1] * 8 <= 96 * 1024:
        return _LayerNormFused.apply(x, gamma, beta, eps)
    return F.layer_norm(x, (x.shape[-1],), gamma, beta, eps)
```

### b200ddp/ops/modules.py

```python
from __future__ import annotations

import math
import os
from typing import Optional

import torch
import torch.nn as nn

from . import functional as Fn


class Linear(nn.Module):

    def __init__(self, in_features: int, out_features: int, bias: bool = True, activation: Optional[str] = None,
                 device=None, dtype=None, fp8: bool = False):
        super().__init__()
        if fp8 and (in_features % 16 or out_features % 16):
            raise ValueError(f"fp8 Linear needs in_features and out_features divisible by 16, got {in_features} -> {out_features}")
        self.in_features, self.out_features, self.activation = in_features, out_features, activation
        self.fp8 = bool(fp8)
        self.weight = nn.Parameter(torch.empty(out_features, in_features, device=device, dtype=dtype))
        self.bias = nn.Parameter(torch.empty(out_features, device=device, dtype=dtype)) if bias else None
        self.reset_parameters()

    def reset_parameters(self) -> None:
        nn.init.kaiming_uniform_(self.weight, a=math.sqrt(5))
        if self.bias is not None:
            bound = 1 / math.sqrt(self.in_features) if self.in_features > 0 else 0
            nn.init.uniform_(self.bias, -bound, bound)

    def forward(self, x: torch.Tensor) -> torch.Tensor:
        return Fn.linear(x, self.weight, self.bias, self.activation, fp8=self.fp8)

    def extra_repr(self) -> str:
        return (f"in={self.in_features}, out={self.out_features}, bias={self.bias is not None}, act={self.activation}"
                + (", fp8=True" if self.fp8 else ""))


class Conv2dTC(nn.Conv2d):

    def __init__(self, in_channels: int, out_channels: int, kernel_size: int = 1, stride: int = 1, **kw):
        super().__init__(in_channels, out_channels, kernel_size, stride=stride, padding=(kernel_size - 1) // 2, bias=False, **kw)

    def _native(self, x: torch.Tensor) -> bool:
        return self.stride[0] == self.stride[1] and Fn.conv_tc_wanted(x, self.weight, self.stride[0], self.padding[0])

    def forward(self, x: torch.Tensor) -> torch.Tensor:
        if self._native(x):
            return Fn.conv2d_tc(x, self.weight, False)[0]
        return super().forward(x)

    def forward_with_stats(self, x: torch.Tensor):
        if self._native(x):
            return Fn.conv2d_tc(x, self.weight, True)
        return super().forward(x), None


class PointwiseConv2d(Conv2dTC):
    def __init__(self, in_channels: int, out_channels: int, stride: int = 1, **kw):
        super().__init__(in_channels, out_channels, 1, stride=stride, **kw)


class Conv3x3(Conv2dTC):
    def __init__(self, in_channels: int, out_channels: int, stride: int = 1, **kw):
        super().__init__(in_channels, out_channels, 3, stride=stride, **kw)


class StemConv7x7(nn.Conv2d):

    def __init__(self, in_channels: int = 3, out_channels: int = 64, **kw):
        super().__init__(in_channels, out_channels, 7, stride=2, padding=3, bias=False, **kw)

    def _native(self, x: torch.Tensor) -> bool:
        return Fn.stem_conv_supported(x, self.weight, self.stride, self.padding)

    def forward(self, x: torch.Tensor) -> torch.Tensor:
        if self._native(x):
            return Fn.stem_conv(x, self.weight, False)[0]
        return super().forward(x)

    def forward_with_stats(self, x: torch.Tensor):
        if self._native(x):
            return Fn.stem_conv(x, self.weight, True)
        return super().forward(x), None


class LayerNorm(nn.Module):
    def __init__(self, hidden: int, eps: float = 1e-5, device=None, dtype=None):
        super().__init__()
        self.eps = eps
        self.weight = nn.Parameter(torch.ones(hidden, device=device, dtype=dtype))
        self.bias = nn.Parameter(torch.zeros(hidden, device=device, dtype=dtype))

    def forward(self, x: torch.Tensor) -> torch.Tensor:
        return Fn.layer_norm(x, self.weight, self.bias, self.eps)


class RMSNorm(nn.Module):

    def __init__(self, hidden: int, eps: float = 1e-5, device=None, dtype=None):
        super().__init__()
        self.eps = eps
        self.weight = nn.Parameter(torch.ones(hidden, device=device, dtype=dtype))

    def forward(self, x: torch.Tensor) -> torch.Tensor:
        return Fn.rms_norm(x, self.weight, self.eps)


class MSELoss(nn.Module):
    def forward(self, out: torch.Tensor, target: torch.Tensor) -> torch.Tensor:
        return Fn.mse_loss(out, target)


class CrossEntropyLoss(nn.Module):
    def __init__(self, ignore_index: int = -100):
        super().__init__()
        self.ignore_index = ignore_index

    def forward(self, logits: torch.Tensor, target: torch.Tensor) -> torch.Tensor:
        return Fn.cross_entropy(logits, target, self.ignore_index)
```

Baseline: 5034 samples/s.

## Overlap wgmma with stage release, dual consumer groups, fused residual-add dgrad epilogue

The conv tap-GEMM kernel gains a second consumer warpgroup that alternates tiles with the first, so one group's MMA can overlap the other's epilogue. It also keeps one wgmma group in flight (wait<1>) and frees ring slots one step late. The epilogue is rewritten to work straight from registers, with a shuffle reduce-scatter for BN stats and a TMA-loaded addend for fused residual adds. On the Python side, dgrad of identity-shortcut conv1 folds the shortcut gradient into the native kernel, and the dgrad policy becomes shape-based. These add register and shared-memory pressure and barrier complexity, and change which convs go through native versus library kernels.

```diff
diff --git a/b200ddp/csrc/conv_wgmma.cu b/b200ddp/csrc/conv_wgmma.cu
--- a/b200ddp/csrc/conv_wgmma.cu
+++ b/b200ddp/csrc/conv_wgmma.cu
@@ -14,16 +14,20 @@
 
 constexpr int BLOCK_K = 64;
 constexpr int UMMA_K = 16;
-constexpr int kThreads = 256;
 constexpr int kMmaWarps = 4;
 constexpr int kMaxRing = 12;
 constexpr int kSlabBytes = 128 * 128;
-constexpr int kStagingBytes = 2 * kSlabBytes;
 constexpr int kBarrierBytes = 1024;
 constexpr int kTrStride = 36;
 constexpr int kStatsScratchBytes = 4 * 32 * kTrStride * 4;
 __host__ __device__ constexpr int acc_stride(int block_n) { return block_n + 8; }
 __host__ __device__ constexpr int acc_bytes(int block_n) { return 128 * acc_stride(block_n) * 4; }
+__host__ __device__ constexpr int num_consumers(int epi) { return epi == 2 ? 1 : 2; }
+__host__ __device__ constexpr int num_threads(int epi) { return 128 * (1 + num_consumers(epi)); }
+__host__ __device__ constexpr int staging_bytes(int block_n, int epi) { return epi == 2 ? 2 * kSlabBytes : num_consumers(epi) * (block_n / 64) * kSlabBytes; }
+__host__ __device__ constexpr int scratch_bytes(int block_n, int epi) {
+  return epi == 1 ? num_consumers(epi) * 4 * 2 * block_n * 4 : epi == 2 ? kStatsScratchBytes + acc_bytes(block_n) : 0;
+}
 
 struct TapGemmParams {
   int M_total, Kc, Nc;
@@ -58,7 +62,25 @@
       ::"r"(smem_u32(smem)), "l"(reinterpret_cast<uint64_t>(map)), "r"(smem_u32(bar)), "r"(c0), "r"(c1), "r"(c2), "r"(c3) : "memory");
 }
 __device__ __forceinline__ void bulk_wait_read_all() { asm volatile("cp.async.bulk.wait_group.read 0;" ::: "memory"); }
-__device__ __forceinline__ void epi_bar_sync() { asm volatile("bar.sync 1, 128;" ::: "memory"); }
+__device__ __forceinline__ void named_bar_sync(int id, int count) { asm volatile("bar.sync %0, %1;" ::"r"(id), "r"(count) : "memory"); }
+__device__ __forceinline__ void named_bar_arrive(int id, int count) { asm volatile("bar.arrive %0, %1;" ::"r"(id), "r"(count) : "memory"); }
+
+template <int M, int H>
+__device__ __forceinline__ void reduce_scatter_step(float* v, int lane) {
+  const bool up = (lane & M) != 0;
+#pragma unroll
+  for (int i = 0; i < H; ++i) {
+    const float send = up ? v[i] : v[i + H];
+    const float keep = up ? v[i + H] : v[i];
+    v[i] = keep + __shfl_xor_sync(0xffffffffu, send, M);
+  }
+}
+template <int N>
+__device__ __forceinline__ void reduce_scatter_8lanes(float* v, int lane) {
+  reduce_scatter_step<16, N / 2>(v, lane);
+  reduce_scatter_step<8, N / 4>(v, lane);
+  reduce_scatter_step<4, N / 8>(v, lane);
+}
 
 __device__ __forceinline__ uint64_t make_desc_rowoff(uint32_t addr, uint32_t lbo, uint32_t sbo, int set_base_offset) {
   uint64_t d = make_smem_desc(addr, lbo, sbo);
@@ -95,22 +117,24 @@
 }
 
 template <int BLOCK_N, bool B_MN, int EPI>
-__global__ void __launch_bounds__(kThreads, 1)
+__global__ void __launch_bounds__(num_threads(EPI), 1)
 conv_tap_gemm_kernel(const __grid_constant__ CUtensorMap map_a, const __grid_constant__ CUtensorMap map_b,
-                     const __grid_constant__ CUtensorMap map_d, const TapGemmParams p) {
+                     const __grid_constant__ CUtensorMap map_d, const __grid_constant__ CUtensorMap map_add, const TapGemmParams p) {
   constexpr int kBBytes = BLOCK_N * BLOCK_K * 2;
   constexpr int kAccStride = acc_stride(BLOCK_N);
+  constexpr int kCons = num_consumers(EPI);
   extern __shared__ uint8_t smem_raw[];
   uint8_t* smem = reinterpret_cast<uint8_t*>((reinterpret_cast<uintptr_t>(smem_raw) + 1023) & ~uintptr_t(1023));
   uint8_t* s_ring = smem;
   uint8_t* b_ring = s_ring + p.s_stages * p.s_stage_bytes;
   uint8_t* staging = b_ring + p.b_stages * p.b_slot_bytes;
-  [[maybe_unused]] float* stats_scratch = reinterpret_cast<float*>(staging + kStagingBytes);
-  float* acc_smem = reinterpret_cast<float*>(staging + kStagingBytes + (EPI != 0 ? kStatsScratchBytes : 0));
-  uint64_t* s_full = reinterpret_cast<uint64_t*>(reinterpret_cast<uint8_t*>(acc_smem) + acc_bytes(BLOCK_N));
+  [[maybe_unused]] float* stats_scratch = reinterpret_cast<float*>(staging + staging_bytes(BLOCK_N, EPI));
+  [[maybe_unused]] float* acc_smem = stats_scratch + kStatsScratchBytes / 4;
+  uint64_t* s_full = reinterpret_cast<uint64_t*>(staging + staging_bytes(BLOCK_N, EPI) + scratch_bytes(BLOCK_N, EPI));
   uint64_t* s_empty = s_full + kMaxRing;
   uint64_t* b_full = s_empty + kMaxRing;
   uint64_t* b_empty = b_full + kMaxRing;
+  uint64_t* add_full = b_empty + kMaxRing;
 
   const int warp = threadIdx.x >> 5, lane = threadIdx.x & 31;
   const long long t_begin = clock64();
@@ -125,6 +149,7 @@
       mbar_init(&s_full[lane], (p.mode == 2 || p.b_resident) ? 1 : 2); mbar_init(&s_empty[lane], kMmaWarps);
       mbar_init(&b_full[lane], 1); mbar_init(&b_empty[lane], kMmaWarps);
     }
+    if (lane < 2) mbar_init(&add_full[lane], 1);
     asm volatile("fence.mbarrier_init.release.cluster;" ::: "memory");
   }
   __syncthreads();
@@ -245,23 +270,57 @@
     const uint64_t a_desc0 = make_smem_desc(smem_u32(s_ring), 16, 1024);
     const uint64_t b_desc_s0 = make_smem_desc(smem_u32(s_ring), kLboB, 1024);
     const uint64_t b_desc_b0 = make_smem_desc(smem_u32(b_ring), kLboB, 1024);
-    const int ew = warp - 4;
-    const bool t0 = (ew == 0 && lane == 0);
-    int ss = 0, bs = 0;
-    uint32_t sph = 0, bph = 0, slab = 0;
+    const int g = (warp >> 2) - 1;
+    const int wt = threadIdx.x - 128 * (g + 1);
+    const int ew = wt >> 5;
+    const bool t0 = (wt == 0);
+    const int local_tiles = (num_tiles - (int)blockIdx.x + (int)gridDim.x - 1) / (int)gridDim.x;
+    const int s_per_tile = p.mode != 2 ? chunks_per_tile / p.KC : cblocks;
+    const int b_per_tile = p.mode == 2 ? cblocks * (taps / p.TB) : 0;
+    uint32_t slab = 0;
     long long d_wf = 0, d_mma = 0, d_ep = 0, t = 0;
-    const bool dbg = p.dbg != nullptr && blockIdx.x == 0 && t0;
-    [[maybe_unused]] float st_s[BLOCK_N / 32], st_q[BLOCK_N / 32];
-    constexpr bool STATS = (EPI != 0);
+    const bool dbg = p.dbg != nullptr && blockIdx.x == 0 && t0 && g == 0;
+    constexpr bool STATS = (EPI == 1 || EPI == 2);
+    uint32_t add_ph = 0;
+    [[maybe_unused]] float st[2 * (BLOCK_N / 32)];
     [[maybe_unused]] float* tr = stats_scratch + ew * (32 * kTrStride);
-    if constexpr (STATS) {
-#pragma unroll
-      for (int i = 0; i < BLOCK_N / 32; ++i) { st_s[i] = 0.f; st_q[i] = 0.f; }
+    [[maybe_unused]] float* st_slot = nullptr;
+    if constexpr (EPI == 1) {
+      const int base = ((lane >> 4) & 1) * 4 + ((lane >> 3) & 1) * 2 + ((lane >> 2) & 1);
+      st_slot = stats_scratch + ((g * 4 + ew) * 2 + ((base >> 1) & 1)) * BLOCK_N + 8 * (base >> 2) + 2 * (lane & 3) + (base & 1);
+#pragma unroll
+      for (int G = 0; G < BLOCK_N / 16; ++G) st_slot[16 * G] = 0.f;
+    }
+    if constexpr (EPI == 2) {
+#pragma unroll
+      for (int i = 0; i < 2 * (BLOCK_N / 32); ++i) st[i] = 0.f;
     }
     if (p.b_resident) mbar_wait(&b_full[0], 0);
-    for (int tile = blockIdx.x; tile < num_tiles; tile += gridDim.x) {
+    for (int L = g; L < local_tiles; L += kCons) {
+      const int tile = (int)blockIdx.x + L * (int)gridDim.x;
+      if constexpr (EPI == 3) {
+        const int mt = tile / p.num_n_tiles, n0 = (tile - mt * p.num_n_tiles) * BLOCK_N;
+        const int row0 = p.mode == 0 ? mt * 128 : (((mt / p.tiles_h) * p.BI) * p.H + (mt % p.tiles_h) * p.BH) * p.W;
+        if (ew == 0) {
+          if (t0) bulk_wait_read_all();
+          __syncwarp();
+          if (elect_one()) {
+            uint8_t* stg = staging + g * (BLOCK_N / 64) * kSlabBytes;
+            const bool two = BLOCK_N == 128 && n0 + 64 < p.Nc;
+            mbar_expect_tx(&add_full[g], (uint32_t)((two ? 2 : 1) * 128 * p.dense_rows));
+            tma_load_2d(&map_add, &add_full[g], stg, n0, row0);
+            if (two) tma_load_2d(&map_add, &add_full[g], stg + kSlabBytes, n0 + 64, row0);
+          }
+          __syncwarp();
+        }
+      }
+      const int s_seq = L * s_per_tile, b_seq = L * b_per_tile;
+      int ss = s_seq % p.s_stages, bs = p.mode == 2 ? b_seq % p.b_stages : 0;
+      uint32_t sph = (uint32_t)(s_seq / p.s_stages) & 1u, bph = p.mode == 2 ? (uint32_t)(b_seq / p.b_stages) & 1u : 0u;
+      if (kCons == 2 && L > 0) named_bar_sync(3 + g, 256);
       WgAcc<BLOCK_N> acc;
       uint32_t acc_on = 0;
+      int prev_s = -1, prev_b = -1;
       if (p.mode != 2) {
         for (int q0 = 0; q0 < chunks_per_tile; q0 += p.KC) {
           B200_T0 mbar_wait(&s_full[ss], sph); B200_T1(d_wf)
@@ -281,9 +340,10 @@
             off += (uint32_t)p.chunk_stride;
           }
           wgmma_commit();
-          wgmma_wait<0>();
+          wgmma_wait<1>();
           __syncwarp();
-          if (lane == 0) mbar_arrive(&s_empty[ss]);
+          if (lane == 0 && prev_s >= 0) mbar_arrive(&s_empty[prev_s]);
+          prev_s = ss;
           if (++ss == p.s_stages) { ss = 0; sph ^= 1; }
           B200_T1(d_mma)
         }
@@ -309,17 +369,26 @@
               if (++sx == p.S) { sx = 0; ++r; }
             }
             wgmma_commit();
-            wgmma_wait<0>();
+            wgmma_wait<1>();
             __syncwarp();
             if (lane == 0) {
-              mbar_arrive(&b_empty[bs]);
-              if (tap0 + p.TB >= taps) mbar_arrive(&s_empty[ss]);
+              if (prev_b >= 0) mbar_arrive(&b_empty[prev_b]);
+              if (prev_s >= 0) mbar_arrive(&s_empty[prev_s]);
             }
+            prev_b = bs;
+            prev_s = (tap0 + p.TB >= taps) ? ss : -1;
             if (++bs == p.b_stages) { bs = 0; bph ^= 1; }
             B200_T1(d_mma)
           }
           if (++ss == p.s_stages) { ss = 0; sph ^= 1; }
         }
+      }
+      if (kCons == 2 && L + 1 < local_tiles) named_bar_arrive(3 + (g ^ 1), 256);
+      wgmma_wait<0>();
+      __syncwarp();
+      if (lane == 0) {
+        if (prev_b >= 0) mbar_arrive(&b_empty[prev_b]);
+        if (prev_s >= 0) mbar_arrive(&s_empty[prev_s]);
       }
       B200_T0
       const int mt = tile / p.num_n_tiles, nt = tile - mt * p.num_n_tiles;
@@ -327,37 +396,83 @@
       int row0;
       if (p.mode == 0) row0 = mt * 128;
       else row0 = (((mt / p.tiles_h) * p.BI) * p.H + (mt % p.tiles_h) * p.BH) * p.W;
-      int dense;
-      bool valid = acc_row_to_dense(p, ew * 32 + lane, &dense);
-      valid = valid && (row0 + dense < p.M_total);
-      wg_bar_sync();
-      acc_to_smem<BLOCK_N>(acc, acc_smem, kAccStride, threadIdx.x - 128);
-      wg_bar_sync();
-#pragma unroll
-      for (int c = 0; c < BLOCK_N; c += 64) {
-        if (n0 + c >= p.Nc) break;
-        uint8_t* buf = staging + (slab & 1u) * kSlabBytes;
-        const uint32_t buf_s = smem_u32(buf);
-#pragma unroll
-        for (int half = 0; half < 2; ++half) {
-          uint32_t rr[32];
-          acc_row_ld32(acc_smem, kAccStride, ew * 32 + lane, c + 32 * half, rr);
+      if constexpr (EPI != 2) {
+        uint8_t* stg = staging + g * (BLOCK_N / 64) * kSlabBytes;
+        const uint32_t stg_s = smem_u32(stg);
+        int dense[2][2];
+        bool valid[2][2];
+#pragma unroll
+        for (int half = 0; half < 2; ++half)
+#pragma unroll
+          for (int hi = 0; hi < 2; ++hi) {
+            valid[half][hi] = acc_row_to_dense(p, 64 * half + 16 * ew + (lane >> 2) + 8 * hi, &dense[half][hi]);
+            valid[half][hi] = valid[half][hi] && (row0 + dense[half][hi] < p.M_total);
+          }
+        if (t0) bulk_wait_read_all();
+        named_bar_sync(1 + g, 128);
+        if constexpr (EPI == 3) { mbar_wait(&add_full[g], add_ph); add_ph ^= 1u; }
+#pragma unroll
+        for (int G = 0; G < BLOCK_N / 16; ++G) {
+          [[maybe_unused]] float sv[8];
+#pragma unroll
+          for (int jj = 0; jj < 2; ++jj) {
+            const int j = 2 * G + jj;
+            if constexpr (EPI == 1) { sv[4 * jj] = 0.f; sv[4 * jj + 1] = 0.f; sv[4 * jj + 2] = 0.f; sv[4 * jj + 3] = 0.f; }
+#pragma unroll
+            for (int half = 0; half < 2; ++half)
+#pragma unroll
+              for (int hi = 0; hi < 2; ++hi) {
+                const int d = dense[half][hi];
+                const uint32_t addr = stg_s + (uint32_t)((j >> 3) * kSlabBytes + d * 128 + (((j & 7) ^ (d & 7)) << 4) + (lane & 3) * 4);
+                float v0 = acc.h[half][4 * j + 2 * hi], v1 = acc.h[half][4 * j + 2 * hi + 1];
+                if constexpr (EPI == 3) {
+                  if (valid[half][hi]) {
+                    uint32_t a;
+                    asm volatile("ld.shared.b32 %0, [%1];" : "=r"(a) : "r"(addr) : "memory");
+                    const float2 f = __bfloat1622float2(*reinterpret_cast<const __nv_bfloat162*>(&a));
+                    v0 += f.x; v1 += f.y;
+                  }
+                }
+                const __nv_bfloat162 h2 = __floats2bfloat162_rn(v0, v1);
+                if (valid[half][hi]) {
+                  asm volatile("st.shared.b32 [%0], %1;" ::"r"(addr), "r"(*reinterpret_cast<const uint32_t*>(&h2)) : "memory");
+                }
+                if constexpr (EPI == 1) {
+                  const float2 f = __bfloat1622float2(h2);
+                  const float x0 = valid[half][hi] ? f.x : 0.f, x1 = valid[half][hi] ? f.y : 0.f;
+                  sv[4 * jj] += x0; sv[4 * jj + 1] += x1; sv[4 * jj + 2] += x0 * x0; sv[4 * jj + 3] += x1 * x1;
+                }
+              }
+          }
           if constexpr (EPI == 1) {
-            float sv[32], qv[32];
-#pragma unroll
-            for (int i = 0; i < 32; ++i) {
-              const float v = __bfloat162float(__float2bfloat16_rn(__uint_as_float(rr[i])));
-              sv[i] = valid ? v : 0.f;
-              qv[i] = sv[i] * sv[i];
-            }
-            const float cs = warp_column_sum32(sv, tr, lane);
-            const float cq = warp_column_sum32(qv, tr, lane);
-            const int ci = (c >> 5) + half;
-#pragma unroll
-            for (int i = 0; i < BLOCK_N / 32; ++i)
-              if (i == ci) { st_s[i] += cs; st_q[i] += cq; }
-          }
-          if constexpr (EPI == 2) {
+            reduce_scatter_8lanes<8>(sv, lane);
+            st_slot[16 * G] += sv[0];
+          }
+        }
+        fence_async_smem();
+        named_bar_sync(1 + g, 128);
+        if (t0) {
+#pragma unroll
+          for (int c = 0; c < BLOCK_N / 64; ++c)
+            if (n0 + 64 * c < p.Nc) tma_store_2d(&map_d, stg + c * kSlabBytes, n0 + 64 * c, row0);
+          bulk_commit();
+        }
+      } else {
+        int dense;
+        bool valid = acc_row_to_dense(p, ew * 32 + lane, &dense);
+        valid = valid && (row0 + dense < p.M_total);
+        named_bar_sync(1, 128);
+        acc_to_smem<BLOCK_N>(acc, acc_smem, kAccStride, wt);
+        named_bar_sync(1, 128);
+#pragma unroll
+        for (int c = 0; c < BLOCK_N; c += 64) {
+          if (n0 + c >= p.Nc) break;
+          uint8_t* buf = staging + (slab & 1u) * kSlabBytes;
+          const uint32_t buf_s = smem_u32(buf);
+#pragma unroll
+          for (int half = 0; half < 2; ++half) {
+            uint32_t rr[32];
+            acc_row_ld32(acc_smem, kAccStride, ew * 32 + lane, c + 32 * half, rr);
             const int col0 = n0 + c + 32 * half;
             const size_t grow = (size_t)(row0 + dense);
             float v[32];
@@ -408,49 +523,52 @@
               const int ci = (c >> 5) + half;
 #pragma unroll
               for (int i = 0; i < BLOCK_N / 32; ++i)
-                if (i == ci) { st_s[i] += cs; st_q[i] += cq; }
+                if (i == ci) { st[2 * i] += cs; st[2 * i + 1] += cq; }
             }
-          }
-          if (valid) {
-#pragma unroll
-            for (int q = 0; q < 4; ++q) {
-              __nv_bfloat162 h[4];
-#pragma unroll
-              for (int j = 0; j < 4; ++j) h[j] = __floats2bfloat162_rn(__uint_as_float(rr[8 * q + 2 * j]), __uint_as_float(rr[8 * q + 2 * j + 1]));
-              const int chunk = half * 4 + q;
-              const uint32_t* w = reinterpret_cast<const uint32_t*>(h);
-              asm volatile("st.shared.v4.b32 [%0], {%1, %2, %3, %4};"
-                           ::"r"(buf_s + (uint32_t)(dense * 128 + ((chunk ^ (dense & 7)) << 4))), "r"(w[0]), "r"(w[1]), "r"(w[2]), "r"(w[3]) : "memory");
+            if (valid) {
+#pragma unroll
+              for (int q = 0; q < 4; ++q) {
+                __nv_bfloat162 h[4];
+#pragma unroll
+                for (int j = 0; j < 4; ++j) h[j] = __floats2bfloat162_rn(__uint_as_float(rr[8 * q + 2 * j]), __uint_as_float(rr[8 * q + 2 * j + 1]));
+                const int chunk = half * 4 + q;
+                const uint32_t* w = reinterpret_cast<const uint32_t*>(h);
+                asm volatile("st.shared.v4.b32 [%0], {%1, %2, %3, %4};"
+                             ::"r"(buf_s + (uint32_t)(dense * 128 + ((chunk ^ (dense & 7)) << 4))), "r"(w[0]), "r"(w[1]), "r"(w[2]), "r"(w[3]) : "memory");
+              }
             }
           }
-        }
-        fence_async_smem();
-        if (t0) bulk_wait_read_all();
-        epi_bar_sync();
-        if (t0) { tma_store_2d(&map_d, buf, n0 + c, row0); bulk_commit(); }
-        ++slab;
+          fence_async_smem();
+          if (t0) bulk_wait_read_all();
+          named_bar_sync(1, 128);
+          if (t0) { tma_store_2d(&map_d, buf, n0 + c, row0); bulk_commit(); }
+          ++slab;
+        }
       }
       B200_T1(d_ep)
     }
     if (dbg) { p.dbg[5] = d_wf; p.dbg[6] = d_mma; p.dbg[9] = d_ep; }
     if (STATS && p.col_stats != nullptr) {
       float* comb = stats_scratch;
-      epi_bar_sync();
-#pragma unroll
-      for (int i = 0; i < BLOCK_N / 32; ++i) {
-        comb[(ew * 2 + 0) * BLOCK_N + 32 * i + lane] = st_s[i];
-        comb[(ew * 2 + 1) * BLOCK_N + 32 * i + lane] = st_q[i];
+      if constexpr (EPI == 2) {
+        named_bar_sync(1, 128);
+#pragma unroll
+        for (int i = 0; i < BLOCK_N / 32; ++i) {
+          comb[(ew * 2 + 0) * BLOCK_N + 32 * i + lane] = st[2 * i];
+          comb[(ew * 2 + 1) * BLOCK_N + 32 * i + lane] = st[2 * i + 1];
+        }
       }
-      epi_bar_sync();
+      named_bar_sync(5, 128 * kCons);
       const int nt = blockIdx.x % p.num_n_tiles;
-      const size_t g = (size_t)(blockIdx.x / p.num_n_tiles), G = (size_t)(gridDim.x / p.num_n_tiles);
-      for (int j = ew * 32 + lane; j < 2 * BLOCK_N; j += 128) {
+      const size_t gi = (size_t)(blockIdx.x / p.num_n_tiles), G = (size_t)(gridDim.x / p.num_n_tiles);
+      for (int j = (int)threadIdx.x - 128; j < 2 * BLOCK_N; j += 128 * kCons) {
         const int which = j / BLOCK_N, cc = j - which * BLOCK_N;
         const int col = nt * BLOCK_N + cc;
         if (col < p.Nc) {
-          const float v = ((comb[(0 * 2 + which) * BLOCK_N + cc] + comb[(1 * 2 + which) * BLOCK_N + cc]) + comb[(2 * 2 + which) * BLOCK_N + cc]) +
-                          comb[(3 * 2 + which) * BLOCK_N + cc];
-          p.col_stats[((size_t)which * G + g) * p.Nc + col] = v;
+          float v = comb[which * BLOCK_N + cc];
+#pragma unroll
+          for (int q = 1; q < kCons * 4; ++q) v += comb[(q * 2 + which) * BLOCK_N + cc];
+          p.col_stats[((size_t)which * G + gi) * p.Nc + col] = v;
         }
       }
     }
@@ -590,9 +708,10 @@
 namespace {
 
 template <int BLOCK_N, bool B_MN, int EPI>
-void launch_variant(const CUtensorMap& ma, const CUtensorMap& mb, const CUtensorMap& md, TapGemmParams p, int want_kc, cudaStream_t stream) {
+void launch_variant(const CUtensorMap& ma, const CUtensorMap& mb, const CUtensorMap& md, const CUtensorMap& madd, TapGemmParams p, int want_kc,
+                    cudaStream_t stream) {
   constexpr int kBBytes = BLOCK_N * BLOCK_K * 2;
-  const int budget = 227 * 1024 - kStagingBytes - kBarrierBytes - 1024 - (EPI != 0 ? kStatsScratchBytes : 0) - acc_bytes(BLOCK_N);
+  const int budget = 227 * 1024 - staging_bytes(BLOCK_N, EPI) - scratch_bytes(BLOCK_N, EPI) - kBarrierBytes - 1024;
   const int taps = p.R * p.S;
   if (p.mode != 2) {
     const int chunks_per_tile = (p.Kc / BLOCK_K) * taps;
@@ -628,13 +747,13 @@
     if (b_st < 2) throw std::runtime_error("conv: shared memory budget exceeded");
     p.s_stages = s_st; p.b_stages = b_st;
   }
-  const int smem = p.s_stages * p.s_stage_bytes + p.b_stages * p.b_slot_bytes + kStagingBytes + kBarrierBytes + 1024 + (EPI != 0 ? kStatsScratchBytes : 0) +
-                   acc_bytes(BLOCK_N);
+  const int smem = p.s_stages * p.s_stage_bytes + p.b_stages * p.b_slot_bytes + staging_bytes(BLOCK_N, EPI) + scratch_bytes(BLOCK_N, EPI) +
+                   kBarrierBytes + 1024;
   auto kernel = conv_tap_gemm_kernel<BLOCK_N, B_MN, EPI>;
   static std::atomic<unsigned long long> configured{0};
   ensure_max_dynamic_smem(kernel, 227 * 1024, configured);
-  const int grid = conv_grid_size(p.num_m_tiles, p.num_n_tiles, EPI != 0);
-  kernel<<<grid, kThreads, smem, stream>>>(ma, mb, md, p);
+  const int grid = conv_grid_size(p.num_m_tiles, p.num_n_tiles, EPI == 1 || EPI == 2);
+  kernel<<<grid, num_threads(EPI), smem, stream>>>(ma, mb, md, madd, p);
   B200_CUDA_CHECK(cudaGetLastError()); B200_COUNT_LAUNCH(1);
 }
 
@@ -705,12 +824,21 @@
     uint32_t bx[2] = {64, (uint32_t)pl.dense_rows};
     md = conv_encode_map(d, 2, dm, st, bx);
   }
+  CUtensorMap madd = md;
+  if (fuse != nullptr && fuse->addend != nullptr && fuse->bn_x == nullptr) {
+    uint64_t dm[2] = {(uint64_t)Nc, (uint64_t)M_total};
+    uint64_t st[1] = {(uint64_t)Nc * 2};
+    uint32_t bx[2] = {64, (uint32_t)pl.dense_rows};
+    madd = conv_encode_map(fuse->addend, 2, dm, st, bx);
+  }
 #define B200_CONV_DISPATCH(BN)                                                                         \
   if (block_n == BN) {                                                                                 \
-    if (dgrad && fuse != nullptr) launch_variant<BN, true, 2>(ma, mb, md, p, cfg.kc, stream);          \
-    else if (dgrad) launch_variant<BN, true, 0>(ma, mb, md, p, cfg.kc, stream);                        \
-    else if (col_stats != nullptr) launch_variant<BN, false, 1>(ma, mb, md, p, cfg.kc, stream);        \
-    else launch_variant<BN, false, 0>(ma, mb, md, p, cfg.kc, stream);                                  \
+    if (dgrad && fuse != nullptr && fuse->bn_x == nullptr)                                             \
+      launch_variant<BN, true, 3>(ma, mb, md, madd, p, cfg.kc, stream);                                \
+    else if (dgrad && fuse != nullptr) launch_variant<BN, true, 2>(ma, mb, md, madd, p, cfg.kc, stream); \
+    else if (dgrad) launch_variant<BN, true, 0>(ma, mb, md, madd, p, cfg.kc, stream);                  \
+    else if (col_stats != nullptr) launch_variant<BN, false, 1>(ma, mb, md, madd, p, cfg.kc, stream);  \
+    else launch_variant<BN, false, 0>(ma, mb, md, madd, p, cfg.kc, stream);                            \
     return;                                                                                            \
   }
   B200_CONV_DISPATCH(64)
@@ -765,8 +893,8 @@
     uint32_t bx[2] = {64, (uint32_t)g.Wo};
     md = conv_encode_map(y, 2, dm, st, bx);
   }
-  if (col_stats != nullptr) launch_variant<64, false, 1>(ma, mb, md, p, 0, stream);
-  else launch_variant<64, false, 0>(ma, mb, md, p, 0, stream);
-}
-
-}
+  if (col_stats != nullptr) launch_variant<64, false, 1>(ma, mb, md, md, p, 0, stream);
+  else launch_variant<64, false, 0>(ma, mb, md, md, p, 0, stream);
+}
+
+}
diff --git a/b200ddp/csrc/conv_wgrad_wgmma.cu b/b200ddp/csrc/conv_wgrad_wgmma.cu
--- a/b200ddp/csrc/conv_wgrad_wgmma.cu
+++ b/b200ddp/csrc/conv_wgrad_wgmma.cu
@@ -138,6 +138,8 @@
     WgAcc<TILE_N> acc;
     int as = 0, bs = 0;
     uint32_t aph = 0, bph = 0;
+    int prev_as = -1, prev_bs = -1;
+    bool prev_frees_a = false;
     for (int kb = kb0; kb < kb1; ++kb) {
       mbar_wait(&a_full[as], aph);
       for (int t = 0; t < ntaps; ++t) {
@@ -150,16 +152,18 @@
           wgmma_tile<TILE_N, 1, 1>(acc, da0 + step, da0 + half_a + step, db0 + step, (kb != kb0 || k != 0) ? 1u : 0u);
         }
         wgmma_commit();
-        wgmma_wait<0>();
+        wgmma_wait<1>();
         __syncwarp();
-        if (lane == 0) {
-          mbar_arrive(&b_empty[bs]);
-          if (t == ntaps - 1) mbar_arrive(&a_empty[as]);
+        if (lane == 0 && prev_bs >= 0) {
+          mbar_arrive(&b_empty[prev_bs]);
+          if (prev_frees_a) mbar_arrive(&a_empty[prev_as]);
         }
+        prev_as = as; prev_bs = bs; prev_frees_a = (t == ntaps - 1);
         if (++bs == p.b_stages) { bs = 0; bph ^= 1; }
       }
       if (++as == p.a_stages) { as = 0; aph ^= 1; }
     }
+    wgmma_wait<0>();
     const int row_len = taps * p.Cin;
     float* out = p.partial + (size_t)sp * p.Cout * row_len + (size_t)co0 * row_len + (size_t)tap0 * p.Cin + ci0;
 #pragma unroll
@@ -249,11 +253,11 @@
   p.b_slot_bytes = (tile_n / 64) * chunk;
   const int budget = 227 * 1024 - kBarrierBytes - 1024;
   int ast = budget / (p.a_slot_bytes + TG * p.b_slot_bytes);
-  if (ast < 1) ast = 1;
+  if (ast < 2) ast = 2;
   if (ast > kMaxRing) ast = kMaxRing;
   int bst = (budget - ast * p.a_slot_bytes) / p.b_slot_bytes;
   if (bst > kMaxRing) bst = kMaxRing;
-  if (bst < 1) return false;
+  if (bst < 2) return false;
   p.a_stages = ast;
   p.b_stages = bst;
   out->p = p;
@@ -386,6 +390,8 @@
     WgAcc<64> acc[kStemGroups];
     int as = 0, bs = 0;
     uint32_t aph = 0, bph = 0;
+    int prev_as = -1, prev_bs = -1;
+    bool prev_frees_b = false;
     for (int kb = kb0; kb < kb1; ++kb) {
       mbar_wait(&b_full[bs], bph);
 #pragma unroll
@@ -399,16 +405,18 @@
           wgmma_tile<64, 1, 1>(acc[g], da0 + step, da0 + half_a + step, db0 + step, (kb != kb0 || k != 0) ? 1u : 0u);
         }
         wgmma_commit();
-        wgmma_wait<0>();
+        wgmma_wait<1>();
         __syncwarp();
-        if (lane == 0) {
-          mbar_arrive(&a_empty[as]);
-          if (g == kStemGroups - 1) mbar_arrive(&b_empty[bs]);
+        if (lane == 0 && prev_as >= 0) {
+          mbar_arrive(&a_empty[prev_as]);
+          if (prev_frees_b) mbar_arrive(&b_empty[prev_bs]);
         }
+        prev_as = as; prev_bs = bs; prev_frees_b = (g == kStemGroups - 1);
         if (++as == p.a_stages) { as = 0; aph ^= 1; }
       }
       if (++bs == p.b_stages) { bs = 0; bph ^= 1; }
     }
+    wgmma_wait<0>();
     float* base = p.partial + (size_t)sp * kStemK * p.Cout;
 #pragma unroll
     for (int g = 0; g < kStemGroups; ++g)
diff --git a/b200ddp/models/resnet.py b/b200ddp/models/resnet.py
--- a/b200ddp/models/resnet.py
+++ b/b200ddp/models/resnet.py
@@ -27,11 +27,11 @@
         if os.environ.get("B200DDP_BLOCK_FUSE", "0") == "1" and bottleneck_native_ok(self, x):
             return bottleneck_forward(self, x)
         if self.downsample is None:
-            identity = x
+            y, part, identity = self.conv1.forward_with_stats_and_shortcut(x)
         else:
             y, part = self.downsample[0].forward_with_stats(x)
             identity = self.downsample[1](y, partials=part)
-        y, part = self.conv1.forward_with_stats(x)
+            y, part = self.conv1.forward_with_stats(x)
         out = self.bn1(y, partials=part)
         y, part = self.conv2.forward_with_stats(out)
         out = self.bn2(y, partials=part)
diff --git a/b200ddp/ops/functional.py b/b200ddp/ops/functional.py
--- a/b200ddp/ops/functional.py
+++ b/b200ddp/ops/functional.py
@@ -594,8 +594,13 @@
     return False
 
 
-def _dgrad_native(cin: int, cout: int, k: int, pixels: int) -> bool:
-    return _conv_policy() == "native"
+def _dgrad_native(cin: int, cout: int, k: int, pixels: int, shortcut: bool = False) -> bool:
+    mode = _conv_policy()
+    if mode != "auto":
+        return mode == "native"
+    if shortcut and k == 1 and pixels >= 25088:
+        return True
+    return pixels >= 100352 and cout <= 128 and (k == 3 or cin >= 256)
 
 
 def _wgrad_native(cin: int, cout: int, k: int, pixels: int) -> bool:
@@ -616,11 +621,12 @@
             and x.shape[1] % 64 == 0 and weight.shape[0] % 64 == 0 and x.shape[3] + 2 <= 256 and _conv_policy() != "lib")
 
 
-def conv_tc_wanted(x: torch.Tensor, weight: torch.Tensor, stride: int, padding: int) -> bool:
+def conv_tc_wanted(x: torch.Tensor, weight: torch.Tensor, stride: int, padding: int, shortcut: bool = False) -> bool:
     if not conv_tc_supported(x, weight, stride, padding):
         return False
     n, cin, h, w = x.shape
-    return _fprop_native(cin, weight.shape[0], weight.shape[2], n * h * w)
+    shape = (cin, weight.shape[0], weight.shape[2], n * h * w)
+    return _fprop_native(*shape) or _dgrad_native(*shape, shortcut)
 
 
 def _cl(t: torch.Tensor) -> torch.Tensor:
@@ -630,21 +636,25 @@
 class _ConvTC(torch.autograd.Function):
 
     @staticmethod
-    def forward(ctx, x, w, want_stats):
+    def forward(ctx, x, w, want_stats, shortcut=False):
         C = _C()
         xc, wc = _cl(x), _cl(w)
         k = w.shape[2]
-        y, st = C.conv_fprop(xc, wc, 1, (k - 1) // 2, -1, 0, 0, bool(want_stats))
+        n, cin, h, wd = x.shape
+        if _fprop_native(cin, w.shape[0], k, n * h * wd):
+            y, st = C.conv_fprop(xc, wc, 1, (k - 1) // 2, -1, 0, 0, bool(want_stats))
+        else:
+            y, st = F.conv2d(xc, wc, None, 1, (k - 1) // 2), None
         ctx.save_for_backward(xc, wc)
         ctx.k = k
         ctx.w_strides = w.stride()
-        if want_stats:
+        ctx.shortcut = shortcut
+        if st is not None:
             ctx.mark_non_differentiable(st)
-            return y, st
-        return y, None
-
-    @staticmethod
-    def backward(ctx, dy, _dstats):
+        return y, st, (x.view_as(x) if shortcut else None)
+
+    @staticmethod
+    def backward(ctx, dy, _dstats, dshort=None):
         C = _C()
         x, w = ctx.saved_tensors
         k = ctx.k
@@ -653,11 +663,16 @@
         dx = dw = None
         n, cin, h, wd = x.shape
         if ctx.needs_input_grad[0]:
-            if _dgrad_native(cin, w.shape[0], k, n * h * wd):
-                dx = C.conv_dgrad(dyc, w, 1, pad, -1, 0, 0)[0]
+            if _dgrad_native(cin, w.shape[0], k, n * h * wd, ctx.shortcut):
+                if dshort is not None:
+                    dx = C.conv_dgrad(dyc, w, 1, pad, -1, 0, 0, 0, _cl(dshort))[0]
+                else:
+                    dx = C.conv_dgrad(dyc, w, 1, pad, -1, 0, 0)[0]
             else:
                 dx = torch.ops.aten.convolution_backward(dyc, x, w, None, [1, 1], [pad, pad], [1, 1], False, [0, 0], 1,
                                                          [True, False, False])[0]
+                if dshort is not None:
+                    dx = dx + dshort
         if ctx.needs_input_grad[1]:
             if _wgrad_native(cin, w.shape[0], k, n * h * wd):
                 dw = C.conv_wgrad(dyc, x, k, 1, pad, 0, 0, 0)
@@ -666,11 +681,11 @@
                                                          [False, True, False])[1]
             if k == 1 and tuple(dw.stride()) != tuple(ctx.w_strides):
                 dw = dw.as_strided(dw.shape, ctx.w_strides)
-        return dx, dw, None
-
-
-def conv2d_tc(x: torch.Tensor, weight: torch.Tensor, want_stats: bool = False):
-    return _ConvTC.apply(x, weight, want_stats)
+        return dx, dw, None, None
+
+
+def conv2d_tc(x: torch.Tensor, weight: torch.Tensor, want_stats: bool = False, shortcut: bool = False):
+    return _ConvTC.apply(x, weight, want_stats, shortcut)
 
 
 def _stem_policy() -> str:
@@ -698,10 +713,9 @@
         ctx.save_for_backward(xp)
         ctx.hw = (int(x.shape[2]), int(x.shape[3]))
         ctx.w_strides = w.stride()
-        if want_stats:
+        if st is not None:
             ctx.mark_non_differentiable(st)
-            return y, st
-        return y, None
+        return y, st
 
     @staticmethod
     def backward(ctx, dy, _dstats):
diff --git a/b200ddp/ops/modules.py b/b200ddp/ops/modules.py
--- a/b200ddp/ops/modules.py
+++ b/b200ddp/ops/modules.py
@@ -42,8 +42,8 @@
     def __init__(self, in_channels: int, out_channels: int, kernel_size: int = 1, stride: int = 1, **kw):
         super().__init__(in_channels, out_channels, kernel_size, stride=stride, padding=(kernel_size - 1) // 2, bias=False, **kw)
 
-    def _native(self, x: torch.Tensor) -> bool:
-        return self.stride[0] == self.stride[1] and Fn.conv_tc_wanted(x, self.weight, self.stride[0], self.padding[0])
+    def _native(self, x: torch.Tensor, shortcut: bool = False) -> bool:
+        return self.stride[0] == self.stride[1] and Fn.conv_tc_wanted(x, self.weight, self.stride[0], self.padding[0], shortcut)
 
     def forward(self, x: torch.Tensor) -> torch.Tensor:
         if self._native(x):
@@ -52,8 +52,13 @@
 
     def forward_with_stats(self, x: torch.Tensor):
         if self._native(x):
-            return Fn.conv2d_tc(x, self.weight, True)
+            return Fn.conv2d_tc(x, self.weight, True)[:2]
         return super().forward(x), None
+
+    def forward_with_stats_and_shortcut(self, x: torch.Tensor):
+        if self._native(x, shortcut=True):
+            return Fn.conv2d_tc(x, self.weight, True, True)
+        return super().forward(x), None, x
 
 
 class PointwiseConv2d(Conv2dTC):
```

New measurement: 5139 samples/s (median of 6 runs). +2.1%, better.
